# blink97/raytracing-gpu

Measured on AMD Instinct MI355X. Metric: Mrays/sec (primary+shadow) at 3840x2160, higher is better.
Workload: dtype f32; 1 GPU; C5 synthetic 10M-triangle sphere field (32x32 UV spheres of 53 stacks x 94 slices = 9776 tris + ground quad, seed 0x5EED, BASELINE.md), 3840x2160, device-built octree, exact camera rays (per-frame candidate lists); width=3840, height=2160, triangles=10010626, accel=octree_gpu

## Files before the change

### raytracing-gpu_amd/csrc/rt_ctx.h

```cpp
#pragma once
#include <hip/hip_runtime.h>
#include <rccl/rccl.h>

#include <algorithm>
#include <cerrno>
#include <chrono>
#include <cmath>
#include <cstdio>
#include <cstdlib>
#include <cstring>
#include <string>
#include <thread>
#include <vector>

#include "rt_build.h"
#include "rt_cand.h"
#include "rt_kernels.h"
#include "rt_forecast.h"
#include "rt_lightbuf.h"
#include "rt_mem.h"
#include "rt_relight.h"
#include "rt_shadow.h"
#include "rt_reflect.h"
#include "rt_tiles.h"

extern "C" {
#include "../host/rt_cull.h"
#include "../host/rt_internal.h"
}

#ifndef RT_EPS_ULPS_DEFAULT
#define RT_EPS_ULPS_DEFAULT 64
#endif
#ifndef RT_OOB_CAP
#define RT_OOB_CAP (1u << 20)
#endif
#ifndef RT_CAM_EPS_ULPS_DEFAULT
#define RT_CAM_EPS_ULPS_DEFAULT 64
#endif

#define HIP_TRY(expr)                                                                    \
  do {                                                                                   \
    hipError_t e_ = (expr);                                                              \
    if (e_ != hipSuccess)                                                                \
      return rt_set_error(RT_EHIP, "%s: %s (%s:%d)", #expr, hipGetErrorString(e_), __FILE__, \
                          __LINE__);                                                     \
  } while (0)

#define RT_TIMED_FRAMES 1024

static constexpr size_t kItemCounterBytes = 8 * 128;
static constexpr size_t kStatBytes = RT_STAT_SETS * RT_STAT_STRIDE * sizeof(unsigned long long);
static constexpr size_t kHitCounterBytes = 2 * RT_HIT_REGIONS * RT_HIT_STRIDE * sizeof(uint32_t);
static constexpr size_t kCostBytes = 64;
static constexpr size_t kFrameCounterBytes =
    kItemCounterBytes + kStatBytes + kHitCounterBytes + kCostBytes;

struct StreamOwner {
  hipStream_t s = nullptr;
  StreamOwner() = default;
  StreamOwner(const StreamOwner&) = delete;
  ~StreamOwner() { if (s) (void)hipStreamDestroy(s); }
  operator hipStream_t() const { return s; }
};

struct rt_hip_ctx {
  int device = 0;
  int accel = RT_ACCEL_FLAT;
  int count_work = 0;
  int grid = 0;
  StreamOwner stream;
  hipStream_t last_stream = nullptr;
  DevBuf<float4> d_tri;
  DevBuf<float> d_nrm;
  DevBuf<float> d_mat;
  DevBuf<float> d_light;
  DevBuf<float4> d_node;
  DevBuf<uint32_t> d_counter;
  unsigned long long* d_stats = nullptr;
  DevBuf<uint2> d_spill;
  uint32_t nrec = 0, nlight = 0;
  rt_accel_info info{};
  float scene_c[3]{}, scene_r = 0;
  float scene_lo[3]{}, scene_hi[3]{};
  float eps_ulps = RT_EPS_ULPS_DEFAULT;
  float cam_eps_ulps = RT_CAM_EPS_ULPS_DEFAULT;
  int policy = RT_POLICY_DEFAULT;
  DevBuf<unsigned long long> d_tile_cycles;
  DevBuf<float4> d_hit;
  DevBuf<uint32_t> d_hit_prev;
  DevBuf<float4> d_hit_term;
  uint32_t* d_hit_count = nullptr;
  size_t hit_cap() const {
    return std::min({d_hit.cap() / 2, d_hit_prev.cap(), d_hit_term.cap()}) / RT_HIT_REGIONS;
  }
  size_t hit_need = 0;
  DevBuf<uint32_t> d_last;
  int gbuffer = 0;
  DevBuf<uint4> d_capture;
  int gb_valid = 0;
  rt_frame gb_frame{};
  int keep_visibility = 0;
  DevBuf<uint32_t> d_hit_lit;
  RelightPlan relight;
  int rl_valid = 0;
  rt_frame rl_frame{};
  std::vector<float> mat_host;
#ifndef RT_ASYNC_LISTS_DEFAULT
#define RT_ASYNC_LISTS_DEFAULT 1
#endif
  int grid_of[2][RT_NPOLICIES][2] = {};
  int cus = 0;
  std::vector<uint32_t> light_type;
  std::vector<float> light_v;
  int light_buffers = 1;
  std::vector<LBDevice*> lb_dev;
  DevBuf<RtLightBuf> d_lbuf;
  std::vector<RtLightBuf> lb_host;
  std::vector<uint8_t> lb_failed;
  float lb_ulps = -1.0f;
  int lb_proven = -1;
  unsigned long long lb_entry_cap = 0;
  KParams last_p{};
  DevBuf<float2> d_prim_mu;
  DevBuf<float2> d_node_mu;
  DevBuf<uint4> d_oob;
  DevBuf<uint32_t> d_oob_count;
  DevBuf<unsigned long long> d_frame_check;
  DevBuf<uint32_t> d_sh_global;
  uint32_t n_sh_global = 0;
  int exact_refl = 0;
  DevBuf<float4> d_node_rf;
  unsigned long long rf_unbounded = 0;
  float sh_ulps = -1.0f;
  float sh_omax = 0.0f;
  float sh_mu_max = 1.0f;
  int exact_shadows = 1;
  size_t tile_cycles_n = 0;
  int exact_camera = 1;
#ifndef RT_CAND_REFINE_DEFAULT
#define RT_CAND_REFINE_DEFAULT 1
#endif
  int cand_refine = RT_CAND_REFINE_DEFAULT;
  const uint32_t* d_cand_valid = nullptr;
  double bound_scale = 1.0;
  float4* d_tri_prim = nullptr;
  DevBuf<float4> d_tri_prim_own;
  uint32_t nprim = 0;
  DevBuf<uint32_t> d_cand_list;
  DevBuf<void> d_cand_fp;
  DevBuf<uint4> d_cand_sfp;
  int cand_store_fp = 0;
  DevBuf<uint32_t> d_cand_visits;
  DevBuf<uint32_t> d_cand_off;
  DevBuf<uint32_t> d_cand_start;
  DevBuf<uint32_t> d_cand_keys;
  DevBuf<uint32_t> d_cand_keys2;
  DevBuf<uint32_t> d_cand_vals;
  DevBuf<uint32_t> d_cand_global;
  DevBuf<uint32_t> d_cand_big;
  DevBuf<uint32_t> d_cand_ctr;
  DevBuf<float> d_cand_skip;
  DevBuf<uint32_t> d_cand_big_lane;
  DevBuf<uint2> d_cand_items;
  DevBuf<uint32_t> d_cand_wave_items;
  DevBuf<uint32_t> d_cand_wave_base;
  DevBuf<uint32_t> d_scan_bsum;
  uint32_t cand_item_cap = 0xffffffffu;
  DevBuf<uint32_t> d_prim_leaf;
  DevBuf<uint32_t> d_cand;
  DevBuf<uint32_t> d_order;
  DevBuf<void> d_scan_tmp;
  PinnedBuf<uint32_t> h_cand;
  int async_lists = RT_ASYNC_LISTS_DEFAULT;
  ListForecast forecast;
  ListShape pknown;
  PinnedBuf<uint32_t> h_kept;
  hipEvent_t ev_kept = nullptr;
  ListShape cost_hist;
  uint32_t cost_waves = 0;
  DevBuf<uint32_t> d_item_cost;
  int last_async = 0;
  unsigned long long cand_prims = 0, cand_entries = 0, cand_global = 0;
  DevBuf<uint32_t> d_send;
  uint32_t send_n = 0;
  DevBuf<uint32_t> d_part;
  DevBuf<uint32_t> d_rstart;
  PinnedBuf<uint32_t> h_rstart;
  KParams ext{};
  int ext_ready = 0, ext_rank = -1, ext_nranks = 0;
  rt_frame ext_frame{};
  uint32_t ext_total = 0;
  int timing = 0;
  hipEvent_t ev[RT_TIMED_FRAMES][5] = {};
  unsigned long long frames = 0;

  ~rt_hip_ctx() {
    for (LBDevice* d : lb_dev) rt_lightbuf_free(d);
    if (ev_kept) (void)hipEventDestroy(ev_kept);
    for (auto& f : ev)
      for (hipEvent_t e : f)
        if (e) (void)hipEventDestroy(e);
  }
};

static inline void lists_changed(rt_hip_ctx* c) {
  c->forecast.reset();
  c->pknown.valid = 0;
}

static inline KParams scene_params(const rt_hip_ctx* c) {
  KParams p;
  std::memset(&p, 0, sizeof p);
  p.tri = c->d_tri;
  p.nrm = c->d_nrm;
  p.mat = c->d_mat;
  p.light = c->d_light;
  p.node = c->d_node;
  p.nrec = c->nrec;
  p.nlight = c->nlight;
  p.tri_prim = c->d_tri_prim;
  p.spill = c->d_spill;
  p.scene_c = rt::f3{c->scene_c[0], c->scene_c[1], c->scene_c[2]};
  p.scene_r = c->scene_r;
  p.scene_cmag = std::fmax(std::fabs(c->scene_c[0]), std::fmax(std::fabs(c->scene_c[1]),
                                                               std::fabs(c->scene_c[2])));
  p.eps_rel = c->eps_ulps * kSlackUnit;
  p.eps_rel_cam = c->cam_eps_ulps * kSlackUnit;
  return p;
}

static inline void scene_extent(const rt_flat_scene& fs, float c[3], float* r) {
  *r = 0;
  for (int a = 0; a < 3; a++) {
    float lo = fs.ntri ? fs.scene_lo[a] : 0.0f, hi = fs.ntri ? fs.scene_hi[a] : 0.0f;
    c[a] = 0.5f * (lo + hi);
    *r = std::fmax(*r, 0.5f * (hi - lo));
  }
}

int shadow_prepare(rt_hip_ctx* c, hipStream_t s);
int lbuf_prepare(rt_hip_ctx* c, hipStream_t s);
int reflect_prepare(rt_hip_ctx* c, hipStream_t s);
int choose_accel(const rt_scene* s);
int cand_prepare(rt_hip_ctx* c, const rt_frame* f, KParams* kp, hipStream_t s, int compat = 0);
unsigned long long* cost_sum_of(rt_hip_ctx* c);
```

### raytracing-gpu_amd/csrc/rt_hip.cpp

```cpp
#include "rt_ctx.h"

extern "C" int rt_hip_tiles_per_rank(int width, int height, int nranks) {
  if (width <= 0 || height <= 0 || nranks <= 0) return 0;
  const int tb = rt_block_side(nranks);
  return (int)(rt_max_rank_blocks((uint32_t)rt_blocks_x(tiles_x_of(width), tb),
                                  (uint32_t)rt_blocks_y(tiles_y_of(height), tb), (uint32_t)nranks) * tb * tb);
}

extern "C" size_t rt_hip_tile_buffer_floats(int width, int height, int nranks) {
  return (size_t)rt_hip_tiles_per_rank(width, height, nranks) * 64 * 3;
}

extern "C" int rt_hip_device_count(int* n) {
  if (!n) return rt_set_error(RT_EINVAL, "null argument");
  int c = 0;
  hipError_t e = hipGetDeviceCount(&c);
  if (e != hipSuccess || c <= 0) {
    *n = 0;
    return rt_set_error(RT_ENODEV, "no HIP device (%s)", hipGetErrorString(e));
  }
  *n = c;
  return RT_OK;
}

template <class T>
static int upload(DevBuf<T>& dst, const void* src, size_t bytes) {
  HIP_TRY(dst.alloc(bytes / sizeof(T)));
  if (src && bytes) HIP_TRY(hipMemcpy(dst, src, bytes, hipMemcpyHostToDevice));
  return RT_OK;
}

extern "C" void rt_hip_destroy(rt_hip_ctx* c) {
  if (!c) return;
  (void)hipSetDevice(c->device);
  delete c;
}

int shadow_prepare(rt_hip_ctx* c, hipStream_t s) {
  if (!c->exact_shadows || c->accel != RT_ACCEL_OCTREE || !c->d_node) return RT_OK;
  if (c->d_node_mu && c->sh_ulps == c->eps_ulps) return RT_OK;
  const size_t np = c->nprim, nn = c->info.nodes;
  if (!c->d_node_mu) {
    HIP_TRY(c->d_prim_mu.alloc(np + 1));
    HIP_TRY(c->d_sh_global.alloc(np + 1));
    HIP_TRY(c->d_node_mu.alloc(nn + 1));
  }
  DevBuf<uint32_t> d_n;
  HIP_TRY(d_n.alloc(1));
  ShadowParams sp;
  std::memset(&sp, 0, sizeof sp);
  sp.tri = c->d_tri_prim;
  sp.nprim = c->nprim;
  sp.light = c->d_light;
  sp.nlight = c->nlight;
  sp.node = c->d_node;
  sp.nnode = (uint32_t)nn;
  sp.rec = c->d_tri;
  for (int a = 0; a < 3; a++) sp.c[a] = c->scene_c[a];
  sp.R = c->scene_r;
  sp.eps_rel = (double)(c->eps_ulps * kSlackUnit);
  const double cmag = std::fmax(std::fabs(c->scene_c[0]), std::fmax(std::fabs(c->scene_c[1]),
                                                                  std::fabs(c->scene_c[2])));
  sp.plane_eps = (double)RT_CULL_PLANE * (cmag + c->scene_r) + 1e-6;
  sp.omax_assumed = 2.0 * c->scene_r + 1.0;
  sp.reach_cap = c->scene_r + 1.0;
  sp.prim_mu = c->d_prim_mu;
  sp.node_mu = c->d_node_mu;
  sp.global = c->d_sh_global;
  sp.nglobal = d_n;
  uint32_t n = 0;
  std::vector<float2> nm(1);
  HIP_TRY(hipMemsetAsync(d_n, 0, sizeof(uint32_t), s));
  HIP_TRY(rt_shadow_build(&sp, (int)c->info.max_depth + 2, s));
  HIP_TRY(hipMemcpyAsync(&n, d_n, sizeof n, hipMemcpyDeviceToHost, s));
  HIP_TRY(hipMemcpyAsync(nm.data(), c->d_node_mu, sizeof(float2), hipMemcpyDeviceToHost, s));
  HIP_TRY(hipStreamSynchronize(s));
  c->n_sh_global = n;
  c->sh_omax = (float)(sp.omax_assumed * (1.0 - 1e-6));
  c->sh_mu_max = nm[0].x;
  c->sh_ulps = c->eps_ulps;
  c->info.shadow_global = n;
  c->info.shadow_mu_max = nm[0].x;
  return RT_OK;
}

static void lbuf_release(rt_hip_ctx* c) {
  for (LBDevice*& d : c->lb_dev) {
    rt_lightbuf_free(d);
    d = nullptr;
  }
  c->d_lbuf.reset();
  c->lb_ulps = -1.0f;
}

static int lbuf_build_one(rt_hip_ctx* c, uint32_t li, hipStream_t s) {
  std::memset(&c->lb_host[li], 0, sizeof(RtLightBuf));
  c->lb_failed[li] = 0;
  const uint32_t t = c->light_type[li];
  if (t != 1 && t != 2) return RT_OK;
  char err[256] = {0};
  LBParams lp;
  lb_fill(lp, c->scene_c, c->scene_r, c->scene_lo, c->scene_hi, c->eps_ulps, t, &c->light_v[3 * li], c->nprim,
          c->exact_shadows);
  lp.tri = c->d_tri_prim;
  lp.max_entries = c->lb_entry_cap;
  if (const char* e = std::getenv("RT_LB_CELLS")) {
    const double k = std::atof(e);
    if (k > 0.0) lp.target_cells = (uint32_t)std::fmin((double)(1u << 26), std::fmax(4096.0, lp.target_cells * k));
  }
  const int br = rt_lightbuf_build(&lp, &c->lb_host[li], &c->lb_dev[li], s, err, sizeof err);
  if (br < 0) {
    (void)hipGetLastError();
    return rt_set_error(RT_EHIP, "light buffer of light %u: %s", li, err);
  }
  if (br > 0) {
    std::memset(&c->lb_host[li], 0, sizeof(RtLightBuf));
    c->lb_dev[li] = nullptr;
    (void)hipGetLastError();
    std::snprintf(c->info.lightbuf_fail_reason, sizeof c->info.lightbuf_fail_reason, "light %u: %s", li, err);
    c->lb_failed[li] = 1;
  }
  return RT_OK;
}

static int lbuf_publish(rt_hip_ctx* c) {
  uint32_t failed = 0;
  for (uint8_t f : c->lb_failed) failed += f;
  c->info.lightbuf_failed = failed;
  if (!failed) c->info.lightbuf_fail_reason[0] = 0;
  if (c->d_lbuf.cap() != c->lb_host.size() || !c->d_lbuf) HIP_TRY(c->d_lbuf.alloc(c->lb_host.size()));
  HIP_TRY(hipMemcpy(c->d_lbuf, c->lb_host.data(), c->lb_host.size() * sizeof(RtLightBuf), hipMemcpyHostToDevice));
  c->lb_ulps = c->eps_ulps;
  c->lb_proven = c->exact_shadows;
  unsigned long long e = 0, n = 0, g = 0, te = 0, tg = 0, nv = 0, bd = 0, tnv = 0, tbd = 0;
  for (LBDevice* d : c->lb_dev) {
    rt_lightbuf_sizes(d, &e, &n, &g);
    rt_lightbuf_proof_counts(d, &nv, &bd);
    te += e;
    tg += g;
    tnv += nv;
    tbd += bd;
  }
  c->info.lightbuf_entries = te;
  c->info.lightbuf_global = tg;
  c->info.lightbuf_never = tnv;
  c->info.lightbuf_band = tbd;
  return RT_OK;
}

int lbuf_prepare(rt_hip_ctx* c, hipStream_t s) {
  if (!c->light_buffers || c->accel != RT_ACCEL_OCTREE || !c->d_node || !c->nlight) return RT_OK;
  if (c->d_lbuf && c->lb_ulps == c->eps_ulps && c->lb_proven == c->exact_shadows) return RT_OK;
  lbuf_release(c);
  c->lb_dev.assign(c->nlight, nullptr);
  c->lb_host.assign(c->nlight, RtLightBuf{});
  c->lb_failed.assign(c->nlight, 0);
  c->info.lightbuf_fail_reason[0] = 0;
  for (uint32_t li = 0; li < c->nlight; li++) {
    const int rc = lbuf_build_one(c, li, s);
    if (rc) {
      for (LBDevice*& d : c->lb_dev) {
        rt_lightbuf_free(d);
        d = nullptr;
      }
      return rc;
    }
  }
  return lbuf_publish(c);
}

extern "C" int rt_hip_set_light_buffers(rt_hip_ctx* c, int enable) {
  if (!c) return rt_set_error(RT_EINVAL, "null context");
  c->light_buffers = enable ? 1 : 0;
  c->relight.invalidate();
  if (!c->light_buffers) lbuf_release(c);
  return RT_OK;
}

extern "C" int rt_hip_set_lightbuf_entry_cap(rt_hip_ctx* c, unsigned long long cap) {
  if (!c) return rt_set_error(RT_EINVAL, "null context");
  c->lb_entry_cap = cap;
  c->relight.invalidate();
  lbuf_release(c);
  HIP_TRY(hipSetDevice(c->device));
  return lbuf_prepare(c, c->stream);
}

extern "C" int rt_hip_create(int device, const rt_scene* scene, int accel, rt_hip_ctx** out) {
  if (!scene || !out) return rt_set_error(RT_EINVAL, "null argument");
  if (accel != RT_ACCEL_FLAT && accel != RT_ACCEL_OCTREE && accel != RT_ACCEL_OCTREE_GPU)
    return rt_set_error(RT_EINVAL, "unknown accel %d", accel);
  const bool dev_build = accel == RT_ACCEL_OCTREE_GPU;
  int ndev = 0;
  int rc = rt_hip_device_count(&ndev);
  if (rc) return rc;
  if (device < 0 || device >= ndev) return rt_set_error(RT_ENODEV, "device %d of %d", device, ndev);
  hipDeviceProp_t prop;
  HIP_TRY(hipGetDeviceProperties(&prop, device));
  if (std::strncmp(prop.gcnArchName, "gfx950", 6) != 0)
    return rt_set_error(RT_ENODEV, "device %d is %s, kernels are built for gfx950", device,
                        prop.gcnArchName);
  HIP_TRY(hipSetDevice(device));

  auto t0 = std::chrono::steady_clock::now();
  rt_flat_scene fs;
  rc = rt_flatten(scene, dev_build ? RT_ACCEL_FLAT : accel, &fs);
  if (rc) return rc;
  auto t1 = std::chrono::steady_clock::now();

  rt_hip_ctx* c = new rt_hip_ctx();
  if (const char* e = std::getenv("RT_CAND_REFINE")) c->cand_refine = std::atoi(e) != 0;
  if (const char* e = std::getenv("RT_ASYNC_LISTS")) c->async_lists = std::atoi(e) != 0;
  c->device = device;
  c->accel = dev_build ? (fs.ntri ? RT_ACCEL_OCTREE : RT_ACCEL_FLAT) : accel;
  c->nrec = (uint32_t)fs.nrec;
  c->nlight = (uint32_t)fs.nlight;
  size_t bytes_tri = fs.nrec * RT_TRI_FLOATS * sizeof(float);
  size_t bytes_nrm = fs.ntri * 9 * sizeof(float);
  size_t bytes_mat = fs.nobj * RT_MAT_FLOATS * sizeof(float);
  size_t bytes_light = fs.nlight * RT_LIGHT_FLOATS * sizeof(float);
  size_t bytes_node = fs.nnode * RT_NODE_FLOATS * sizeof(float);
  rc = upload(c->d_tri, fs.tri, bytes_tri);
  if (!rc) rc = upload(c->d_nrm, fs.nrm, bytes_nrm);
  if (!rc) rc = upload(c->d_mat, fs.mat, bytes_mat);
  if (!rc) rc = upload(c->d_light, fs.light, bytes_light);
  if (!rc && fs.nnode) rc = upload(c->d_node, fs.node, bytes_node);
  if (!rc) rc = upload(c->d_counter, nullptr, kFrameCounterBytes);
  if (!rc) {
    c->d_stats = (unsigned long long*)((char*)c->d_counter.get() + kItemCounterBytes);
    c->d_hit_count = (uint32_t*)((char*)c->d_counter.get() + kItemCounterBytes + kStatBytes);
  }
  if (!rc && hipStreamCreateWithFlags(&c->stream.s, hipStreamNonBlocking) != hipSuccess)
    rc = rt_set_error(RT_EHIP, "hipStreamCreate");
  rt_device_tree tree{};
  if (!rc && dev_build && fs.ntri) {
    rt_device_build_opts o{24, 7};
    if (const char* e = std::getenv("RT_DEV_LEAF")) o.leaf_cap = std::atoi(e);
    if (const char* e = std::getenv("RT_DEV_CLIP")) o.clip_level = std::atoi(e);
    hipError_t he = rt_device_build_octree(c->d_tri, (uint32_t)fs.ntri, fs.scene_lo, fs.scene_hi,
                                           &o, c->stream, &tree);
    if (he != hipSuccess) {
      rc = rt_set_error(RT_EHIP, "device octree build: %s", hipGetErrorString(he));
    } else {
      c->d_tri_prim_own = std::move(c->d_tri);
      c->d_tri_prim = c->d_tri_prim_own;
      c->d_tri.adopt(tree.tri, (size_t)tree.nref * RT_TRI_FLOATS / 4);
      c->d_node.adopt(tree.node, (size_t)tree.nnode * RT_NODE_FLOATS / 4);
      c->nrec = tree.nref;
      bytes_tri = (size_t)tree.nref * RT_TRI_FLOATS * sizeof(float);
      bytes_node = (size_t)tree.nnode * RT_NODE_FLOATS * sizeof(float);
      fs.nrec = tree.nref;
      fs.nnode = tree.nnode;
      fs.leaves = tree.leaves;
      fs.max_depth = tree.depth;
      fs.max_leaf = tree.max_leaf;
    }
  }
  auto t2 = std::chrono::steady_clock::now();
  c->nprim = (uint32_t)fs.ntri;
  if (!rc && !c->d_tri_prim) {
    if (c->accel == RT_ACCEL_FLAT) {
      c->d_tri_prim = c->d_tri;
    } else {
      rt_flat_scene fp;
      rc = rt_flatten(scene, RT_ACCEL_FLAT, &fp);
      if (!rc) {
        rc = upload(c->d_tri_prim_own, fp.tri, fp.nrec * RT_TRI_FLOATS * sizeof(float));
        c->d_tri_prim = c->d_tri_prim_own;
        rt_flat_free(&fp);
      }
    }
  }
  scene_extent(fs, c->scene_c, &c->scene_r);
  for (int a = 0; a < 3; a++) {
    c->scene_lo[a] = fs.ntri ? fs.scene_lo[a] : 0.0f;
    c->scene_hi[a] = fs.ntri ? fs.scene_hi[a] : 0.0f;
  }
  c->info.triangles = fs.ntri;
  c->info.tri_refs = fs.nrec;
  c->info.nodes = fs.nnode;
  c->info.leaves = fs.leaves;
  c->info.max_depth = fs.max_depth;
  c->info.max_leaf = fs.max_leaf;
  c->info.tri_record_bytes = RT_TRI_FLOATS * sizeof(float);
  c->info.node_record_bytes = RT_NODE_FLOATS * sizeof(float);
  c->info.device_bytes = bytes_tri + bytes_nrm + bytes_mat + bytes_light + bytes_node;
  c->info.build_seconds = std::chrono::duration<double>(dev_build ? t2 - t0 : t1 - t0).count();
  if (fs.mat) c->mat_host.assign(fs.mat, fs.mat + fs.nobj * RT_MAT_FLOATS);
  rt_flat_free(&fs);
  if (rc) {
    rt_hip_destroy(c);
    return rc;
  }
  c->grid = prop.multiProcessorCount * 16;
  c->cus = prop.multiProcessorCount;
  for (size_t li = 0; li < scene->light_count; li++) {
    c->light_type.push_back((uint32_t)scene->lights[li].type);
    c->light_v.push_back(scene->lights[li].v.x);
    c->light_v.push_back(scene->lights[li].v.y);
    c->light_v.push_back(scene->lights[li].v.z);
  }
  int gmax = c->grid;
  const int dacc = c->accel == RT_ACCEL_FLAT ? RT_ACCEL_FLAT_D : RT_ACCEL_OCTREE_D;
  for (int tr = 0; tr < 2; tr++)
    for (int pol = 0; pol < RT_NPOLICIES; pol++)
      for (int cw = 0; cw < 2; cw++) {
        int g = 0;
        hipError_t he = rt_render_grid(tr, dacc, cw, pol, prop.multiProcessorCount, &g);
        if (he != hipSuccess) {
          rt_hip_destroy(c);
          return rt_set_error(RT_EHIP, "occupancy query: %s", hipGetErrorString(he));
        }
        c->grid_of[tr][pol][cw] = g;
        gmax = g > gmax ? g : gmax;
      }
  c->info.trace_grid = c->grid_of[1][RT_POLICY_DEFAULT][0];
  c->info.shade_grid = c->grid_of[0][RT_POLICY_LBUF][0];
  for (int a = 0; a < 3; a++) c->info.scene_center[a] = c->scene_c[a];
  c->info.scene_radius = c->scene_r;
  if (c->accel == RT_ACCEL_OCTREE &&
      c->d_spill.alloc((size_t)gmax * 64 * RT_SPILL_STACK) != hipSuccess) {
    rt_hip_destroy(c);
    return rt_set_error(RT_EHIP, "hipMalloc traversal spill stack");
  }
  {
    const auto l0 = std::chrono::steady_clock::now();
    rc = lbuf_prepare(c, c->stream);
    c->info.lightbuf_seconds = std::chrono::duration<double>(std::chrono::steady_clock::now() - l0).count();
    if (rc) {
      rt_hip_destroy(c);
      return rc;
    }
  }
  *out = c;
  return RT_OK;
}

extern "C" int rt_hip_accel_info(const rt_hip_ctx* c, rt_accel_info* out) {
  if (!c || !out) return rt_set_error(RT_EINVAL, "null argument");
  *out = c->info;
  return RT_OK;
}

extern "C" int rt_hip_set_cull_slack(rt_hip_ctx* c, float ulps) {
  if (!c || !(ulps >= 0.0f)) return rt_set_error(RT_EINVAL, "bad slack");
  c->eps_ulps = ulps;
  c->cam_eps_ulps = ulps;
  c->relight.invalidate();
  lists_changed(c);
  return RT_OK;
}

extern "C" int rt_hip_set_camera_slack(rt_hip_ctx* c, float ulps) {
  if (!c || !(ulps >= 0.0f)) return rt_set_error(RT_EINVAL, "bad slack");
  c->cam_eps_ulps = ulps;
  lists_changed(c);
  return RT_OK;
}

extern "C" int rt_hip_set_exact_camera(rt_hip_ctx* c, int enable) {
  if (!c) return rt_set_error(RT_EINVAL, "null context");
  c->exact_camera = enable ? 1 : 0;
  return RT_OK;
}

extern "C" int rt_hip_set_exact_shadows(rt_hip_ctx* c, int enable) {
  if (!c) return rt_set_error(RT_EINVAL, "null context");
  c->exact_shadows = enable ? 1 : 0;
  c->relight.invalidate();
  HIP_TRY(hipSetDevice(c->device));
  int rc = lbuf_prepare(c, c->stream);
  if (rc) return rc;
  if (c->exact_shadows) return shadow_prepare(c, c->stream);
  return RT_OK;
}

static int reflect_build(rt_hip_ctx* c, hipStream_t s) {
  const size_t nn = c->info.nodes;
  DevBuf<float> phi;
  DevBuf<uint32_t> d_u;
  HIP_TRY(c->d_node_rf.alloc(3 * nn + 3));
  HIP_TRY(phi.alloc(nn + 1));
  HIP_TRY(d_u.alloc(1));
  ReflParams rp;
  std::memset(&rp, 0, sizeof rp);
  rp.node = c->d_node;
  rp.nnode = (uint32_t)nn;
  rp.rec = c->d_tri;
  rp.node_rf = c->d_node_rf;
  rp.node_phi = phi;
  rp.unbounded = d_u;
  uint32_t u = 0;
  HIP_TRY(hipMemsetAsync(c->d_node_rf, 0, (3 * nn + 3) * sizeof(float4), s));
  HIP_TRY(hipMemsetAsync(d_u, 0, sizeof(uint32_t), s));
  HIP_TRY(rt_reflect_build(&rp, (int)c->info.max_depth + 2, s));
  HIP_TRY(hipMemcpyAsync(&u, d_u, sizeof u, hipMemcpyDeviceToHost, s));
  HIP_TRY(hipStreamSynchronize(s));
  c->rf_unbounded = u;
  return RT_OK;
}

int reflect_prepare(rt_hip_ctx* c, hipStream_t s) {
  if (c->d_node_rf || c->accel != RT_ACCEL_OCTREE || !c->d_node) return RT_OK;
  const int rc = reflect_build(c, s);
  if (rc) c->d_node_rf.reset();
  return rc;
}

extern "C" int rt_hip_set_exact_reflections(rt_hip_ctx* c, int enable) {
  if (!c) return rt_set_error(RT_EINVAL, "null context");
  c->exact_refl = enable ? 1 : 0;
  if (!c->exact_refl) return RT_OK;
  HIP_TRY(hipSetDevice(c->device));
  return reflect_prepare(c, c->stream);
}

extern "C" int rt_hip_set_policy(rt_hip_ctx* c, int policy) {
  if (!c) return rt_set_error(RT_EINVAL, "null context");
  if (policy < RT_POLICY_DEFAULT || policy > RT_POLICY_DIR_STAGED)
    return rt_set_error(RT_EINVAL, "unknown traversal policy %d", policy);
  c->policy = policy;
  c->relight.invalidate();
  return RT_OK;
}

extern "C" int rt_hip_set_camera_refine(rt_hip_ctx* c, int enable) {
  if (!c) return rt_set_error(RT_EINVAL, "null context");
  c->cand_refine = enable ? 1 : 0;
  lists_changed(c);
  return RT_OK;
}

extern "C" int rt_hip_set_camera_bound_scale(rt_hip_ctx* c, double scale) {
  if (!c || !(scale > 0.0)) return rt_set_error(RT_EINVAL, "bad bound scale");
  c->bound_scale = scale;
  lists_changed(c);
  return RT_OK;
}

static int mask_buffer(rt_hip_ctx* c) {
  const size_t n = c->hit_cap() * RT_HIT_REGIONS;
  if (c->d_hit_lit.holds(n)) return RT_OK;
  c->relight.invalidate();
  HIP_TRY(c->d_hit_lit.alloc(n));
  return RT_OK;
}

static int hit_buffers(rt_hip_ctx* c, size_t ntiles) {
  const size_t items = 4 * ntiles;
  HIP_TRY(c->d_last.grow(items * 64, items * 64));
  if (c->gbuffer) HIP_TRY(c->d_capture.grow(items * 64, items * 64));
  size_t want =(2 * items * 64 + RT_HIT_REGIONS - 1) / RT_HIT_REGIONS + 1024;
  if (c->hit_need > want) want = c->hit_need;
  if (want > (1ull << 29) - 1) want = (1ull << 29) - 1;
  if (want <= c->hit_cap()) return c->keep_visibility ? mask_buffer(c) : RT_OK;
  c->d_hit.reset();
  c->d_hit_prev.reset();
  c->d_hit_term.reset();
  c->d_hit_lit.reset();
  c->relight.invalidate();
  const size_t n = want * RT_HIT_REGIONS;
  HIP_TRY(c->d_hit.alloc(2 * n));
  HIP_TRY(c->d_hit_prev.alloc(n));
  HIP_TRY(c->d_hit_term.alloc(n));
  return c->keep_visibility ? mask_buffer(c) : RT_OK;
}


static int render_refuse(const rt_hip_ctx* c, const rt_frame* f, int rank, int nranks, const float* d_tiles) {
  if (!c || !f || !d_tiles) return rt_set_error(RT_EINVAL, "null argument");
  if (nranks <= 0 || rank < 0 || rank >= nranks)
    return rt_set_error(RT_EINVAL, "rank %d of %d", rank, nranks);
  if (f->width <= 0 || f->height <= 0) return rt_set_error(RT_EINVAL, "empty frame");
  if ((f->width | f->height) & 1)
    return rt_set_error(RT_EINVAL, "frame %dx%d: cpu/rt renders even sizes only", f->width, f->height);
  if (c->gbuffer) {
    if (c->policy != RT_POLICY_DEFAULT)
      return rt_set_error(RT_EINVAL, "the G-buffer needs the default traversal policy (have %d)", c->policy);
    if (c->count_work) return rt_set_error(RT_EINVAL, "the G-buffer cannot be captured by the work-counting pass");
    if (c->exact_refl) return rt_set_error(RT_EINVAL, "the G-buffer cannot be captured with exact reflections on");
  }
  return RT_OK;
}

static void render_frame_params(KParams& p, const rt_hip_ctx* c, const rt_frame* f, int rank, int nranks,
                                float* d_tiles) {
  p.u = rt::f3{f->u.x, f->u.y, f->u.z};
  p.v = rt::f3{f->v.x, f->v.y, f->v.z};
  p.C = rt::f3{f->C.x, f->C.y, f->C.z};
  p.pos = rt::f3{f->position.x, f->position.y, f->position.z};
  p.W = f->width;
  p.H = f->height;
  p.tiles_x = tiles_x_of(f->width);
  p.ntiles_total = tiles_x_of(f->width) * tiles_y_of(f->height);
  p.rank = rank;
  p.nranks = nranks;
  p.ntiles_local = rank_tile_count(f->width, f->height, rank, nranks);
  p.out = d_tiles;
  p.tile_counter = c->d_counter;
  p.stats = c->d_stats;
}

static int render_done(rt_hip_ctx* c, const KParams& p, const rt_frame* f, hipStream_t s, int first_ev) {
  c->last_p = p;
  if (c->gbuffer) {
    c->gb_frame = *f;
    c->gb_valid = 1;
  }
  c->rl_frame = *f;
  c->rl_valid = 1;
  if (p.hit_lit)
    c->relight.masks_written();
  else
    c->relight.invalidate();
  if (c->timing) {
    hipEvent_t* ev = c->ev[c->frames % RT_TIMED_FRAMES];
    for (int k = first_ev; k < 5; k++) HIP_TRY(hipEventRecord(ev[k], s));
    c->frames++;
  }
  c->last_stream = s;
  return RT_OK;
}

static int render_nothing(rt_hip_ctx* c, const KParams& p, const rt_frame* f, hipStream_t s) {
  c->cand_prims = c->cand_entries = c->cand_global = 0;
  c->d_cand_valid = nullptr;
  c->last_async = 0;
  if (c->timing) HIP_TRY(hipEventRecord(c->ev[c->frames % RT_TIMED_FRAMES][0], s));
  HIP_TRY(hipMemsetAsync(c->d_counter, 0, kFrameCounterBytes, s));
  c->cost_hist.valid = 0;
  return render_done(c, p, f, s, 1);
}

static int render_buffers(rt_hip_ctx* c, KParams& p) {
  {
    int rc = hit_buffers(c, (size_t)p.ntiles_local);
    if (rc) return rc;
  }
  if (c->gbuffer) p.capture = c->d_capture;
  if (c->keep_visibility) p.hit_lit = c->d_hit_lit;
  p.hit = c->d_hit;
  p.hit_prev = c->d_hit_prev;
  p.hit_term = c->d_hit_term;
  p.hit_count = c->d_hit_count;
  p.shade_counter = c->d_hit_count + RT_HIT_REGIONS * RT_HIT_STRIDE;
  p.hit_cap = (uint32_t)c->hit_cap();
  p.last = c->d_last;
  if (c->count_work) {
    const size_t items = 4 * (size_t)p.ntiles_local;
    HIP_TRY(c->d_tile_cycles.grow(6 * items, 6 * items));
    c->tile_cycles_n = items;
    p.tile_cycles = c->d_tile_cycles;
  }
  return RT_OK;
}

static int render_shadows(rt_hip_ctx* c, KParams& p, hipStream_t s) {
  {
    int rc = lbuf_prepare(c, s);
    if (rc) return rc;
    if (c->policy == RT_POLICY_DEFAULT || c->policy == RT_POLICY_LANE) p.lbuf = c->d_lbuf;
  }
  const bool walks = !p.lbuf || c->info.lightbuf_failed;
  if (walks) {
    int rc = shadow_prepare(c, s);
    if (rc) return rc;
  }
  if (p.lbuf && c->exact_shadows && c->nlight <= 32) {
    if (!c->d_oob) {
      HIP_TRY(c->d_oob_count.alloc(1));
      HIP_TRY(c->d_oob.alloc(RT_OOB_CAP));
    }
    p.oob = c->d_oob;
    p.oob_count = c->d_oob_count;
    p.oob_cap = RT_OOB_CAP;
    HIP_TRY(hipMemsetAsync(c->d_oob_count, 0, sizeof(uint32_t), s));
  }
  if (c->exact_shadows && walks) {
    p.node_mu = c->d_node_mu;
    p.sh_global = c->d_sh_global;
    p.n_sh_global = c->n_sh_global;
    p.sh_omax = c->sh_omax;
  }
  return RT_OK;
}

static int render_lists(rt_hip_ctx* c, const rt_frame* f, KParams& p, bool use_ext, hipStream_t s) {
  c->cand_prims = c->cand_entries = c->cand_global = 0;
  c->d_cand_valid = nullptr;
  if (c->timing) HIP_TRY(hipEventRecord(c->ev[c->frames % RT_TIMED_FRAMES][0], s));
  if (c->accel == RT_ACCEL_OCTREE && c->d_node && c->exact_camera) {
    if (use_ext) {
      p.cand_start = c->ext.cand_start;
      p.cand = c->ext.cand;
      p.cand_global = c->ext.cand_global;
      p.n_cand_global = c->ext.n_cand_global;
      p.cand_skip = c->ext.cand_skip;
      p.tile_order = c->ext.tile_order;
      p.n_heavy = c->ext.n_heavy;
      p.tri_prim = c->ext.tri_prim;
      c->cand_entries = c->ext_total;
      c->d_cand_valid = nullptr;
      c->cand_global = c->ext.n_cand_global;
      c->cand_prims = 0;
    } else {
      int rc = cand_prepare(c, f, &p, s);
      if (rc) return rc;
    }
  }
  if (!(c->accel == RT_ACCEL_OCTREE && c->d_node && c->exact_camera && !use_ext)) c->last_async = 0;
  return RT_OK;
}

struct RenderKernels {
  int dacc, tpol, spol, gt, gs;
};

static int render_kernels(rt_hip_ctx* c, KParams& p, hipStream_t s, RenderKernels* out) {
  const bool empty = c->accel == RT_ACCEL_OCTREE && !c->d_node;
  const int dacc = (c->accel == RT_ACCEL_FLAT || empty) ? RT_ACCEL_FLAT_D : RT_ACCEL_OCTREE_D;
  const int pol = dacc == RT_ACCEL_FLAT_D ? 0 : c->policy, cw = c->count_work ? 1 : 0;
  int spol = pol;
  if (dacc == RT_ACCEL_OCTREE_D && p.lbuf && !p.node_mu && !p.n_sh_global &&
      (pol == RT_POLICY_DEFAULT || pol == RT_POLICY_LANE)) {
    bool all = true;
    for (uint32_t li = 0; li < c->nlight && all; li++)
      if (c->light_type[li] == 1 || c->light_type[li] == 2) all = c->lb_dev[li] != nullptr;
    if (all) spol = RT_POLICY_LBUF;
  }
  int tpol = pol;
  if (dacc == RT_ACCEL_OCTREE_D && c->exact_refl) {
    if (pol != RT_POLICY_DEFAULT)
      return rt_set_error(RT_EINVAL, "exact reflections need the default traversal policy (have %d)", pol);
    int rc = reflect_prepare(c, s);
    if (rc) return rc;
    p.node_rf = c->d_node_rf;
    tpol = RT_POLICY_EXACT_REFL;
  }
  if (c->gbuffer) tpol = RT_POLICY_GBUFFER;
  int gt = empty ? c->grid : c->grid_of[1][tpol][cw], gs = empty ? c->grid : c->grid_of[0][spol][cw];
  {
    const long long items = 4ll * p.ntiles_local;
    if (items < gt) gt = (int)items;
    if (items < gs) gs = (int)items;
  }
  *out = RenderKernels{dacc, tpol, spol, gt, gs};
  return RT_OK;
}

static int render_launch(rt_hip_ctx* c, const rt_frame* f, int rank, int nranks, KParams& p,
                         const RenderKernels& k, hipStream_t s) {
  hipEvent_t* ev = c->ev[c->frames % RT_TIMED_FRAMES];
  if (!p.tri_prim && (p.lbuf || p.n_sh_global || p.cand_start))
    return rt_set_error(RT_EHIP, "render: prim-order records missing");
  if (!p.hit || !p.last || !p.out || (p.nrec && (!p.tri || !p.nrm)))
    return rt_set_error(RT_EHIP, "render: device buffers missing");
  if (c->gbuffer && !p.capture) return rt_set_error(RT_EHIP, "render: G-buffer capture buffer missing");
  if (p.tile_order) {
    const size_t items = 4 * (size_t)p.ntiles_local;
    if (!c->d_item_cost.holds(items)) {
      c->cost_hist.valid = 0;
      HIP_TRY(c->d_item_cost.grow(items, items));
    }
    p.item_cost = c->d_item_cost;
    p.cost_sum = cost_sum_of(c);
  }
  if (!c->d_frame_check) {
    HIP_TRY(c->d_frame_check.alloc(4));
    HIP_TRY(hipMemsetAsync(c->d_frame_check, 0, 4 * sizeof(unsigned long long), s));
  }
  p.frame_check = c->d_frame_check;
  p.list_flag = c->last_async ? c->d_cand_ctr + RT_CAND_CTR_SNAPSHOT + RT_CC_OVERFLOW : nullptr;
  HIP_TRY(hipMemsetAsync(c->d_counter, 0, kFrameCounterBytes, s));
  if (c->timing) HIP_TRY(hipEventRecord(ev[1], s));
  HIP_TRY(rt_launch_trace(&p, k.dacc, c->count_work, k.tpol, k.gt, s));
  if (p.item_cost) {
    c->cost_hist.set(f, rank, nranks);
    c->cost_waves = (uint32_t)k.gt;
  } else {
    c->cost_hist.valid = 0;
  }
  if (c->timing) HIP_TRY(hipEventRecord(ev[2], s));
  HIP_TRY(rt_launch_shade(&p, k.dacc, c->count_work, k.spol, k.gs, s));
  HIP_TRY(rt_launch_shade_fixup(&p, c->nprim, s));
  if (c->timing) HIP_TRY(hipEventRecord(ev[3], s));
  HIP_TRY(rt_launch_fold(&p, s));
  return RT_OK;
}

extern "C" int rt_hip_render(rt_hip_ctx* c, const rt_frame* f, int rank, int nranks,
                             float* d_tiles, void* stream) {
  int rc = render_refuse(c, f, rank, nranks, d_tiles);
  if (rc) return rc;
  c->gb_valid = 0;
  c->rl_valid = 0;
  HIP_TRY(hipSetDevice(c->device));
  hipStream_t s = stream ? (hipStream_t)stream : c->stream;
  const bool use_ext = c->ext_ready && c->ext_rank == rank && c->ext_nranks == nranks &&
                       std::memcmp(&c->ext_frame, f, sizeof *f) == 0;
  c->ext_ready = 0;
  KParams p = scene_params(c);
  render_frame_params(p, c, f, rank, nranks, d_tiles);
  if (p.ntiles_local == 0) return render_nothing(c, p, f, s);
  RenderKernels k;
  if ((rc = render_buffers(c, p)) || (rc = render_shadows(c, p, s)) || (rc = render_lists(c, f, p, use_ext, s)) ||
      (rc = render_kernels(c, p, s, &k)) || (rc = render_launch(c, f, rank, nranks, p, k, s)))
    return rc;
  return render_done(c, p, f, s, 4);
}

extern "C" int rt_hip_stats(rt_hip_ctx* c, rt_stats* out) {
  if (!c || !out) return rt_set_error(RT_EINVAL, "null argument");
  HIP_TRY(hipSetDevice(c->device));
  unsigned long long hs[RT_STAT_SETS * RT_STAT_STRIDE], h[RT_NSTATS];
  uint32_t hc[RT_HIT_REGIONS * RT_HIT_STRIDE];
  hipStream_t s = c->last_stream ? c->last_stream : c->stream;
  HIP_TRY(hipMemcpyAsync(hs, c->d_stats, sizeof hs, hipMemcpyDeviceToHost, s));
  HIP_TRY(hipMemcpyAsync(hc, c->d_hit_count, sizeof hc, hipMemcpyDeviceToHost, s));
  uint32_t valid = 0, actr[RT_CC_BUILD_WORDS] = {};
  if (c->d_cand_valid) HIP_TRY(hipMemcpyAsync(&valid, c->d_cand_valid, sizeof valid, hipMemcpyDeviceToHost, s));
  const int was_async = c->last_async;
  if (was_async)
    HIP_TRY(hipMemcpyAsync(actr, c->d_cand_ctr + RT_CAND_CTR_SNAPSHOT, sizeof actr, hipMemcpyDeviceToHost, s));
  HIP_TRY(hipStreamSynchronize(s));
  if (c->d_cand_valid) {
    c->cand_entries = valid;
    c->d_cand_valid = nullptr;
  }
  if (was_async) {
    c->last_async = 0;
    c->cand_global = actr[RT_CC_GLOBAL];
    if (actr[RT_CC_OVERFLOW]) {
      lists_changed(c);
      return rt_set_error(RT_EHITBUF, "%u candidate-list entries, %u expected: render again", actr[RT_CC_TOTAL],
                          c->forecast.known.total);
    }
  }
  for (int k = 0; k < RT_NSTATS; k++) {
    h[k] = 0;
    for (int set = 0; set < RT_STAT_SETS; set++) h[k] += hs[set * RT_STAT_STRIDE + k];
  }
  size_t need = 0;
  unsigned long long records = 0;
  for (int x = 0; x < RT_HIT_REGIONS; x++) {
    need = hc[RT_HIT_STRIDE * x] > need ? hc[RT_HIT_STRIDE * x] : need;
    records += hc[RT_HIT_STRIDE * x];
  }
  std::memset(out, 0, sizeof *out);
  for (int k = 0; k < RT_NSTATS; k++) out->*rt_stat_member[k] = h[k];
  out->camera = 4 * h[RT_ST_PIXELS];
  out->hit_records = records;
  out->cand_prims = c->cand_prims;
  out->cand_entries = c->cand_entries;
  out->cand_global = c->cand_global;
  if (need > c->hit_cap()) {
    c->hit_need = need + need / 4 + 1024;
    return rt_set_error(RT_EHITBUF, "%llu hit records, %zu per region held (grown to %zu: render again)",
                        records, c->hit_cap(), c->hit_need);
  }
  if (out->depth_overflow)
    return rt_set_error(RT_EDEPTH, "%llu paths overflowed the bounce limit or a traversal stack",
                        out->depth_overflow);
  if (out->zero_normal)
    return rt_set_error(RT_EZERONORMAL,
                        "%llu closest hits had an exactly zero interpolated normal (cpu/hit.c:79 "
                        "would skip those objects)",
                        out->zero_normal);
  if (out->shadow_zero_risk)
    return rt_set_error(RT_EZERONORMAL,
                        "%llu shadow rays hit an object whose interpolated normal can vanish "
                        "(cpu/hit.c:99 may skip it; early any-hit exit not proven exact)",
                        out->shadow_zero_risk);
  if (c->last_p.oob) {
    uint32_t q = 0;
    HIP_TRY(hipMemcpy(&q, c->d_oob_count, sizeof q, hipMemcpyDeviceToHost));
    out->shadow_deferred = q;
    if (q > RT_OOB_CAP)
      return rt_set_error(RT_EINEXACT, "%u shadow queries from off the exact mode's proof box, %u decided",
                          q, RT_OOB_CAP);
  }
  if (out->closest_unproven)
    return rt_set_error(RT_EINEXACT,
                        "%llu reflection rays with |d| past the exact reflection walk's bound "
                        "(csrc/rt_reflect.h RT_RF_DLMAX)", out->closest_unproven);
  if (out->shadow_unproven)
    return rt_set_error(RT_EINEXACT,
                        "%llu shadow rays left from beyond the extent the exact shadow mode's "
                        "bound assumes (csrc/rt_shadow.hip, csrc/rt_lightbuf.hip)",
                        out->shadow_unproven);
  if (c->accel == RT_ACCEL_OCTREE && c->d_node &&
      (!c->exact_camera || c->bound_scale < 1.0 || c->eps_ulps < RT_EPS_ULPS_DEFAULT))
    return rt_set_error(RT_EINEXACT,
                        "rendered with exact_camera=%d, camera bound scale %g, culling slack %g ulps "
                        "(defaults 1, 1, %d): cpu/rt parity not guaranteed",
                        c->exact_camera, c->bound_scale, (double)c->eps_ulps, RT_EPS_ULPS_DEFAULT);
  return RT_OK;
}

extern "C" int rt_hip_assemble(rt_hip_ctx* c, const rt_frame* f, const float* d_gathered,
                               int nranks, float* d_rgb, void* stream) {
  if (!c || !f || !d_gathered || !d_rgb || nranks <= 0)
    return rt_set_error(RT_EINVAL, "bad argument");
  HIP_TRY(hipSetDevice(c->device));
  hipStream_t s = stream ? (hipStream_t)stream : c->stream;
  int tx = tiles_x_of(f->width);
  int nt = tx * tiles_y_of(f->height);
  HIP_TRY(rt_launch_assemble(d_gathered, d_rgb, f->width, f->height, tx, nt, nranks,
                             rt_hip_tiles_per_rank(f->width, f->height, nranks), s));
  return RT_OK;
}

extern "C" int rt_hip_render_image(rt_hip_ctx* c, const rt_frame* f, float* h_rgb, rt_stats* st) {
  if (!c || !f || !h_rgb) return rt_set_error(RT_EINVAL, "null argument");
  HIP_TRY(hipSetDevice(c->device));
  size_t nt = rt_hip_tile_buffer_floats(f->width, f->height, 1);
  size_t npx = (size_t)f->width * f->height;
  DevBuf<float> d_tiles, d_rgb;
  HIP_TRY(d_tiles.alloc(nt));
  if (d_rgb.alloc(npx * 3) != hipSuccess) return rt_set_error(RT_EHIP, "hipMalloc image");
  rt_stats tmp;
  int rc = RT_OK;
  for (int attempt = 0; attempt < 3; attempt++) {
    rc = rt_hip_render(c, f, 0, 1, d_tiles, nullptr);
    if (!rc) rc = rt_hip_assemble(c, f, d_tiles, 1, d_rgb, nullptr);
    if (!rc && hipMemcpyAsync(h_rgb, d_rgb, npx * 3 * sizeof(float), hipMemcpyDeviceToHost,
                              c->stream) != hipSuccess)
      rc = rt_set_error(RT_EHIP, "D2H image");
    if (!rc) rc = rt_hip_stats(c, st ? st : &tmp);
    if (rc != RT_EHITBUF) break;
  }
  return rc;
}


static std::vector<RelightLight> light_table(const rt_hip_ctx* c) {
  std::vector<RelightLight> t(c->nlight);
  for (uint32_t li = 0; li < c->nlight; li++) t[li] = RelightLight(c->light_type[li], &c->light_v[3 * li]);
  return t;
}

static int relight_quiesce(rt_hip_ctx* c) {
  if (c->last_stream && c->last_stream != c->stream.s) HIP_TRY(hipStreamSynchronize(c->last_stream));
  HIP_TRY(hipStreamSynchronize(c->stream));
  return RT_OK;
}

extern "C" int rt_hip_set_lights(rt_hip_ctx* c, const rt_light* lights, size_t n) {
  if (!c || (n && !lights)) return rt_set_error(RT_EINVAL, "null argument");
  if (n > 0x7fffffffu / RT_LIGHT_FLOATS) return rt_set_error(RT_EINVAL, "%zu lights", n);
  HIP_TRY(hipSetDevice(c->device));
  int rc = relight_quiesce(c);
  if (rc) return rc;
  std::vector<float> rows(n * RT_LIGHT_FLOATS, 0.0f), lv(3 * n);
  std::vector<uint32_t> type(n);
  for (size_t li = 0; li < n; li++) {
    const rt_light& l = lights[li];
    float* L = &rows[RT_LIGHT_FLOATS * li];
    type[li] = (uint32_t)l.type;
    std::memcpy(&L[0], &type[li], sizeof(float));
    L[1] = l.r, L[2] = l.g, L[3] = l.b;
    L[4] = lv[3 * li] = l.v.x, L[5] = lv[3 * li + 1] = l.v.y, L[6] = lv[3 * li + 2] = l.v.z;
  }
  const std::vector<RelightLight> was = light_table(c);
  const size_t old_n = c->nlight;
  rc = upload(c->d_light, rows.data(), rows.size() * sizeof(float));
  if (rc) return rc;
  c->nlight = (uint32_t)n;
  c->light_type = type;
  c->light_v = lv;
  const std::vector<RelightLight> now = light_table(c);
  std::vector<uint8_t> rebuild, release;
  c->relight.set_lights(was, now, rebuild, release);
  bool edited = was.size() != now.size();
  for (size_t li = 0; li < now.size() && !edited; li++) edited = !now[li].same(was[li]);
  if (edited) c->sh_ulps = -1.0f;
  c->last_p.light = c->d_light;
  c->last_p.nlight = c->nlight;
  if (!(c->light_buffers && c->accel == RT_ACCEL_OCTREE && c->d_node)) return RT_OK;
  const bool current = c->d_lbuf && c->lb_ulps == c->eps_ulps && c->lb_proven == c->exact_shadows &&
                       c->lb_dev.size() == old_n && c->lb_host.size() == old_n && c->lb_failed.size() == old_n;
  if (!current || n == 0) {
    lbuf_release(c);
    c->lb_dev.clear();
    c->lb_host.clear();
    c->lb_failed.clear();
    c->last_p.lbuf = nullptr;
    c->info.lightbuf_entries = c->info.lightbuf_global = c->info.lightbuf_never = c->info.lightbuf_band = 0;
    c->info.lightbuf_failed = 0;
    c->info.lightbuf_fail_reason[0] = 0;
    rc = lbuf_prepare(c, c->stream);
    if (c->last_p.hit) c->last_p.lbuf = c->d_lbuf;
    return rc;
  }
  for (size_t li = 0; li < old_n; li++)
    if (release[li]) {
      rt_lightbuf_free(c->lb_dev[li]);
      c->lb_dev[li] = nullptr;
    }
  c->lb_dev.resize(n, nullptr);
  c->lb_host.resize(n, RtLightBuf{});
  c->lb_failed.resize(n, 0);
  for (uint32_t li = 0; li < n; li++) {
    if (!now[li].casts()) {
      c->lb_host[li] = RtLightBuf{};
      c->lb_failed[li] = 0;
    }
    if (!rebuild[li]) continue;
    rc = lbuf_build_one(c, li, c->stream);
    if (rc) {
      lbuf_release(c);
      c->last_p.lbuf = nullptr;
      return rc;
    }
  }
  rc = lbuf_publish(c);
  c->last_p.lbuf = c->last_p.lbuf ? c->d_lbuf.get() : nullptr;
  return rc;
}

extern "C" int rt_hip_set_materials(rt_hip_ctx* c, const rt_object* objects, size_t n) {
  if (!c || (n && !objects)) return rt_set_error(RT_EINVAL, "null argument");
  if (n * RT_MAT_FLOATS != c->mat_host.size())
    return rt_set_error(RT_EINVAL, "%zu objects, the context has %zu", n, c->mat_host.size() / RT_MAT_FLOATS);
  std::vector<float> rows(c->mat_host.size(), 0.0f);
  for (size_t o = 0; o < n; o++) {
    const rt_object& ob = objects[o];
    float* m = &rows[RT_MAT_FLOATS * o];
    m[0] = ob.ka.x, m[1] = ob.ka.y, m[2] = ob.ka.z;
    m[3] = ob.kd.x, m[4] = ob.kd.y, m[5] = ob.kd.z;
    m[6] = ob.ks.x, m[7] = ob.ks.y, m[8] = ob.ks.z;
    m[9] = ob.ns;
    m[10] = ob.nr;
    if (std::memcmp(&m[10], &c->mat_host[RT_MAT_FLOATS * o + 10], 2 * sizeof(float)) != 0)
      return rt_set_error(RT_EINVAL, "object %zu: nr %g differs from the context's %g (reflectivity changes the paths: "
                          "create a new context)", o, (double)ob.nr, (double)c->mat_host[RT_MAT_FLOATS * o + 10]);
  }
  if (!n) return RT_OK;
  HIP_TRY(hipSetDevice(c->device));
  const int rc = relight_quiesce(c);
  if (rc) return rc;
  HIP_TRY(hipMemcpy(c->d_mat, rows.data(), rows.size() * sizeof(float), hipMemcpyHostToDevice));
  c->mat_host = rows;
  return RT_OK;
}

extern "C" int rt_hip_set_keep_visibility(rt_hip_ctx* c, int enable) {
  if (!c) return rt_set_error(RT_EINVAL, "null context");
  c->keep_visibility = enable ? 1 : 0;
  return RT_OK;
}

extern "C" int rt_hip_relight(rt_hip_ctx* c, const rt_frame* f, int rank, int nranks, float* d_tiles,
                              void* stream) {
  if (!c || !f || !d_tiles) return rt_set_error(RT_EINVAL, "null argument");
  if (!c->rl_valid)
    return rt_set_error(RT_EINVAL, "no kept hit records: rt_hip_render first (rt_hip_render_compat keeps none)");
  const KParams& lp = c->last_p;
  if (lp.rank != rank || lp.nranks != nranks || std::memcmp(&c->rl_frame, f, sizeof *f) != 0)
    return rt_set_error(RT_EINVAL, "the kept records are another frame's (last render: %dx%d, rank %d of %d)", lp.W,
                        lp.H, lp.rank, lp.nranks);
  hipStream_t s = stream ? (hipStream_t)stream : c->stream;
  if (s != c->last_stream) return rt_set_error(RT_EINVAL, "a relight runs on the stream of its render");
  if (c->policy != RT_POLICY_DEFAULT)
    return rt_set_error(RT_EINVAL, "a relight needs the default traversal policy (have %d)", c->policy);
  if (c->count_work) return rt_set_error(RT_EINVAL, "a relight cannot run as the work-counting pass");
  if (lp.ntiles_local == 0) return RT_OK;
  HIP_TRY(hipSetDevice(c->device));
  KParams p = lp;
  {
    const KParams sp = scene_params(c);
    p.light = sp.light;
    p.nlight = sp.nlight;
    p.mat = sp.mat;
    p.eps_rel = sp.eps_rel;
    p.eps_rel_cam = sp.eps_rel_cam;
  }
  p.out = d_tiles;
  p.lbuf = nullptr;
  p.node_mu = nullptr;
  p.sh_global = nullptr;
  p.n_sh_global = 0;
  p.sh_omax = 0.0f;
  p.oob = nullptr;
  p.oob_count = nullptr;
  p.oob_cap = 0;
  p.shade_stride = p.shade_first = 0;
  p.relight_dirty = 0;
  p.frame_check = nullptr;
  p.list_flag = nullptr;
  int rc = mask_buffer(c);
  if (rc) return rc;
  p.hit_lit = c->d_hit_lit;
  RenderKernels k;
  if ((rc = render_shadows(c, p, s)) || (rc = render_kernels(c, p, s, &k))) return rc;
  const RelightWork w = c->relight.work(light_table(c));
  if (w.path == RT_RELIGHT_RECOLOUR) p.oob = nullptr;
  if (!p.tri_prim && (p.lbuf || p.n_sh_global)) return rt_set_error(RT_EHIP, "relight: prim-order records missing");
  if (!p.hit || !p.hit_prev || !p.hit_term || !p.hit_lit || !p.hit_count || !p.shade_counter || !p.stats ||
      !p.last || !p.out || (p.nlight && !p.light) || (p.nrec && (!p.tri || !p.nrm)) || !p.mat ||
      p.hit_cap != c->hit_cap() || !c->d_hit_lit.holds((size_t)p.hit_cap * RT_HIT_REGIONS))
    return rt_set_error(RT_EHIP, "relight: device buffers missing");
  HIP_TRY(rt_launch_relight_zero(&p, s));
  if (w.path == RT_RELIGHT_RECOLOUR) {
    HIP_TRY(rt_launch_recolour(&p, c->cus, s));
  } else if (w.path == RT_RELIGHT_PARTIAL) {
    p.relight_dirty = w.dirty;
    HIP_TRY(rt_launch_reshade(&p, k.dacc, k.spol, k.gs, s));
  } else {
    HIP_TRY(rt_launch_shade(&p, k.dacc, 0, k.spol, k.gs, s));
  }
  HIP_TRY(rt_launch_shade_fixup(&p, c->nprim, s));
  HIP_TRY(rt_launch_fold(&p, s));
  c->relight.masks_written();
  c->last_p = p;
  return RT_OK;
}

extern "C" int rt_hip_relight_image(rt_hip_ctx* c, const rt_frame* f, float* h_rgb, rt_stats* st) {
  if (!c || !f || !h_rgb) return rt_set_error(RT_EINVAL, "null argument");
  if (f->width <= 0 || f->height <= 0) return rt_set_error(RT_EINVAL, "empty frame");
  HIP_TRY(hipSetDevice(c->device));
  const size_t nt = rt_hip_tile_buffer_floats(f->width, f->height, 1);
  const size_t npx = (size_t)f->width * f->height;
  DevBuf<float> d_tiles, d_rgb;
  HIP_TRY(d_tiles.alloc(nt));
  if (d_rgb.alloc(npx * 3) != hipSuccess) return rt_set_error(RT_EHIP, "hipMalloc image");
  rt_stats tmp;
  int rc = rt_hip_relight(c, f, 0, 1, d_tiles, nullptr);
  if (rc) return rc;
  rc = rt_hip_assemble(c, f, d_tiles, 1, d_rgb, nullptr);
  if (!rc && hipMemcpyAsync(h_rgb, d_rgb, npx * 3 * sizeof(float), hipMemcpyDeviceToHost, c->stream) != hipSuccess)
    rc = rt_set_error(RT_EHIP, "D2H image");
  const int src = rt_hip_stats(c, st ? st : &tmp);
  return rc ? rc : src;
}

static_assert(RT_GB_WORDS == RT_GB_WORDS_D && sizeof(rt_gsample) == 4 * RT_GB_WORDS,
              "rt_gsample is the record gbuffer_kernel writes");
extern "C" int rt_hip_set_gbuffer(rt_hip_ctx* c, int enable) {
  if (!c) return rt_set_error(RT_EINVAL, "null context");
  c->gbuffer = enable ? 1 : 0;
  if (!c->gbuffer) c->gb_valid = 0;
  return RT_OK;
}

extern "C" size_t rt_hip_gbuffer_tile_words(int width, int height, int nranks) {
  return (size_t)rt_hip_tiles_per_rank(width, height, nranks) * 64 * 4 * RT_GB_WORDS;
}

extern "C" int rt_hip_gbuffer(rt_hip_ctx* c, const rt_frame* f, int rank, int nranks, void* d_tiles,
                              void* stream) {
  if (!c || !f || !d_tiles) return rt_set_error(RT_EINVAL, "null argument");
  if ((uintptr_t)d_tiles & 7) return rt_set_error(RT_EINVAL, "G-buffer tiles must be 8-byte aligned");
  if (!c->gbuffer || !c->gb_valid)
    return rt_set_error(RT_EINVAL, "no G-buffer capture: rt_hip_set_gbuffer(1), then rt_hip_render");
  const KParams& lp = c->last_p;
  if (lp.rank != rank || lp.nranks != nranks || std::memcmp(&c->gb_frame, f, sizeof *f) != 0)
    return rt_set_error(RT_EINVAL, "the G-buffer holds another frame (last render: %dx%d, rank %d of %d)",
                        lp.W, lp.H, lp.rank, lp.nranks);
  hipStream_t s = stream ? (hipStream_t)stream : c->stream;
  if (s != c->last_stream)
    return rt_set_error(RT_EINVAL, "the G-buffer must be read on the stream of its render");
  if (lp.ntiles_local == 0) return RT_OK;
  HIP_TRY(hipSetDevice(c->device));
  if (!lp.capture || !lp.hit || (lp.nrec && !lp.tri_prim))
    return rt_set_error(RT_EHIP, "G-buffer: device buffers missing");
  HIP_TRY(rt_launch_gbuffer(&lp, (uint32_t*)d_tiles, s));
  return RT_OK;
}

extern "C" int rt_hip_assemble_gbuffer(rt_hip_ctx* c, const rt_frame* f, const void* d_gathered, int nranks,
                                       void* d_samples, void* stream) {
  if (!c || !f || !d_gathered || !d_samples || nranks <= 0) return rt_set_error(RT_EINVAL, "bad argument");
  if (f->width <= 0 || f->height <= 0) return rt_set_error(RT_EINVAL, "empty frame");
  HIP_TRY(hipSetDevice(c->device));
  hipStream_t s = stream ? (hipStream_t)stream : c->stream;
  HIP_TRY(rt_launch_assemble_words((const uint32_t*)d_gathered, (uint32_t*)d_samples, f->width, f->height,
                                   tiles_x_of(f->width), nranks,
                                   rt_hip_tiles_per_rank(f->width, f->height, nranks), 4 * RT_GB_WORDS, s));
  return RT_OK;
}

extern "C" int rt_hip_render_image_gbuffer(rt_hip_ctx* c, const rt_frame* f, float* h_rgb,
                                           rt_gsample* h_samples, rt_stats* st) {
  if (!c || !f || !h_rgb || !h_samples) return rt_set_error(RT_EINVAL, "null argument");
  if (f->width <= 0 || f->height <= 0) return rt_set_error(RT_EINVAL, "empty frame");
  HIP_TRY(hipSetDevice(c->device));
  const size_t nt = rt_hip_tile_buffer_floats(f->width, f->height, 1);
  const size_t ng = rt_hip_gbuffer_tile_words(f->width, f->height, 1);
  const size_t npx = (size_t)f->width * f->height;
  const size_t nsw = npx * 4 * RT_GB_WORDS;
  DevBuf<float> d_tiles, d_rgb;
  DevBuf<uint32_t> d_gt, d_gs;
  if (d_tiles.alloc(nt) != hipSuccess || d_rgb.alloc(npx * 3) != hipSuccess || d_gt.alloc(ng) != hipSuccess ||
      d_gs.alloc(nsw) != hipSuccess)
    return rt_set_error(RT_EHIP, "hipMalloc image and G-buffer");
  int rc = RT_OK;
  const int was = c->gbuffer;
  c->gbuffer = 1;
  rt_stats tmp;
  for (int attempt = 0; attempt < 3; attempt++) {
    rc = rt_hip_render(c, f, 0, 1, d_tiles, nullptr);
    if (!rc) rc = rt_hip_assemble(c, f, d_tiles, 1, d_rgb, nullptr);
    if (!rc) rc = rt_hip_gbuffer(c, f, 0, 1, d_gt, nullptr);
    if (!rc) rc = rt_hip_assemble_gbuffer(c, f, d_gt, 1, d_gs, nullptr);
    if (!rc && (hipMemcpyAsync(h_rgb, d_rgb, npx * 3 * sizeof(float), hipMemcpyDeviceToHost, c->stream) !=
                    hipSuccess ||
                hipMemcpyAsync(h_samples, d_gs, nsw * sizeof(uint32_t), hipMemcpyDeviceToHost, c->stream) !=
                    hipSuccess))
      rc = rt_set_error(RT_EHIP, "D2H image and G-buffer");
    if (!rc) rc = rt_hip_stats(c, st ? st : &tmp);
    if (rc != RT_EHITBUF) break;
  }
  c->gbuffer = was;
  if (!was) c->gb_valid = 0;
  return rc;
}

int choose_accel(const rt_scene* s);

extern "C" int rt_hip_render_compat(rt_hip_ctx* c, const rt_camera* cam, unsigned char* h_rgba,
                                    rt_stats* st) {
  if (!c || !cam || !h_rgba) return rt_set_error(RT_EINVAL, "null argument");
  if (cam->width <= 0 || cam->height <= 0) return rt_set_error(RT_EINVAL, "empty frame");
  if ((long long)cam->width * cam->height > (1ll << 28) / 9)
    return rt_set_error(RT_EINVAL, "frame too large for the 3x render");
  HIP_TRY(hipSetDevice(c->device));
  rt_camera big = *cam;
  big.width = 3 * cam->width;
  big.height = 3 * cam->height;
  rt_frame f;
  int rc = rt_frame_from_camera_any(&big, &f);
  if (rc) return rc;
  const size_t nhi = (size_t)big.width * big.height, nlo = (size_t)cam->width * cam->height;
  DevBuf<uint32_t> d_hi, d_lo;
  HIP_TRY(d_hi.alloc(nhi));
  if (d_lo.alloc(nlo) != hipSuccess) return rt_set_error(RT_EHIP, "hipMalloc image");
  hipStream_t s = c->stream;
  KParams p = scene_params(c);
  p.u = rt::f3{f.u.x, f.u.y, f.u.z};
  p.v = rt::f3{f.v.x, f.v.y, f.v.z};
  p.C = rt::f3{f.C.x, f.C.y, f.C.z};
  p.pos = rt::f3{f.position.x, f.position.y, f.position.z};
  p.W = big.width;
  p.H = big.height;
  p.tiles_x = tiles_x_of(big.width);
  p.ntiles_total = tiles_x_of(big.width) * tiles_y_of(big.height);
  p.nranks = 1;
  p.ntiles_local = p.ntiles_total;
  p.out = (float*)d_hi.get();
  p.tile_counter = c->d_counter;
  p.stats = c->d_stats;
  const int accel = (c->accel == RT_ACCEL_FLAT || !c->d_node) ? RT_ACCEL_FLAT_D : RT_ACCEL_OCTREE_D;
  rc = shadow_prepare(c, s);
  if (rc) return rc;
  if (c->exact_shadows) {
    p.node_mu = c->d_node_mu;
    p.sh_global = c->d_sh_global;
    p.n_sh_global = c->n_sh_global;
    p.sh_omax = c->sh_omax;
  }
  c->cand_prims = c->cand_entries = c->cand_global = 0;
  c->d_cand_valid = nullptr;
  if (c->accel == RT_ACCEL_OCTREE && c->d_node && c->exact_camera) {
    rc = cand_prepare(c, &f, &p, s, 1);
    if (rc) return rc;
  }
  c->cost_hist.valid = 0;
  c->rl_valid = 0;
  c->relight.invalidate();
  if (hipMemsetAsync(c->d_counter, 0, kFrameCounterBytes, s) != hipSuccess ||
      rt_launch_compat(&p, accel, c->grid, s) != hipSuccess ||
      rt_launch_downscale(d_hi, d_lo, cam->width, cam->height, s) != hipSuccess ||
      hipMemcpyAsync(h_rgba, d_lo, nlo * sizeof(uint32_t), hipMemcpyDeviceToHost, s) != hipSuccess)
    rc = rt_set_error(RT_EHIP, "compat render: %s", hipGetErrorString(hipGetLastError()));
  c->last_stream = s;
  rt_stats tmp;
  if (!rc) rc = rt_hip_stats(c, st ? st : &tmp);
  if (st) st->camera = st->pixels;
  return rc;
}

extern "C" int rt_raytrace_gpu(const char* input, const char* output, int accel) {
  rt_scene* scene = nullptr;
  int rc = rt_scene_load_svati(input, &scene);
  if (rc) return rc;
  if (accel < 0) accel = choose_accel(scene);
  rt_hip_ctx* ctx = nullptr;
  std::vector<unsigned char> img((size_t)4 * (scene->camera.width > 0 ? scene->camera.width : 0) *
                                 (scene->camera.height > 0 ? scene->camera.height : 0) + 4);
  rc = rt_hip_create(0, scene, accel, &ctx);
  if (!rc) rc = rt_hip_render_compat(ctx, &scene->camera, img.data(), nullptr);
  if (!rc) rc = rt_png_write_rgba(output, scene->camera.width, scene->camera.height, img.data());
  if (ctx) rt_hip_destroy(ctx);
  rt_scene_free(scene);
  return rc;
}

extern "C" int rt_hip_malloc(int device, size_t bytes, void** d_ptr) {
  if (!d_ptr) return rt_set_error(RT_EINVAL, "null argument");
  HIP_TRY(hipSetDevice(device));
  HIP_TRY(hipMalloc(d_ptr, bytes ? bytes : 16));
  return RT_OK;
}
extern "C" int rt_hip_free(void* d_ptr) {
  HIP_TRY(hipFree(d_ptr));
  return RT_OK;
}
extern "C" int rt_hip_memcpy_d2h(void* dst, const void* src, size_t bytes) {
  HIP_TRY(hipMemcpy(dst, src, bytes, hipMemcpyDeviceToHost));
  return RT_OK;
}
extern "C" int rt_hip_memcpy_h2d(void* dst, const void* src, size_t bytes) {
  HIP_TRY(hipMemcpy(dst, src, bytes, hipMemcpyHostToDevice));
  return RT_OK;
}

extern "C" int rt_hip_memcpy_d2d(void* dst, const void* src, size_t bytes, void* stream) {
  if (!bytes) return RT_OK;
  HIP_TRY(hipMemcpyAsync(dst, src, bytes, hipMemcpyDeviceToDevice, (hipStream_t)stream));
  return RT_OK;
}


int choose_accel(const rt_scene* s) {
  size_t n = rt_scene_triangle_count(s);
  return n <= 64 ? RT_ACCEL_FLAT : (n < 100000 ? RT_ACCEL_OCTREE : RT_ACCEL_OCTREE_GPU);
}

extern "C" int rt_raytrace(const char* input, const char* output) {
  return rt_raytrace_multi(input, output, 1, -1, nullptr, nullptr);
}
```

### raytracing-gpu_amd/csrc/rt_isect.h

```cpp
#pragma once

#include <hip/hip_runtime.h>
#include <stdint.h>

#include "rt_cull.h"
#include "rt_device.h"
#include "rt_kernels.h"

namespace rt {

static constexpr float kEps = 0.0000001f;

__device__ __forceinline__ void wave_sync() { __asm__ volatile("" ::: "memory"); }
__device__ __forceinline__ uint64_t wave_ballot(bool p) { return __builtin_amdgcn_ballot_w64(p); }

__device__ __forceinline__ f3 ld3(const float* p) { return f3{p[0], p[1], p[2]}; }

__device__ __forceinline__ bool mt_test(f3 o, f3 d, f3 v0, f3 e1, f3 e2, float& t, float& u,
                                        float& v) {
  f3 h = cross(d, e2);
  float a = dot(e1, h);
  if (a > -kEps && a < kEps) return false;
  float f = 1.0f / a;
  f3 s = sub(o, v0);
  u = f * dot(s, h);
  if (u < 0.0f || u > 1.0f) return false;
  f3 q = cross(s, e1);
  v = f * dot(d, q);
  if (v < 0.0f || u + v > 1.0f) return false;
  t = f * dot(e2, q);
  return t > kEps;
}

struct Ray {
  f3 o, d;
  float dlen;
  float eps;
  f3 oh, ol;
};

__device__ __forceinline__ Ray make_ray(const KParams& p, f3 o, f3 d, float eps_rel) {
  Ray r;
  r.o = o;
  r.d = d;
  r.dlen = length(d);
  r.eps = rt_cull_eps(eps_rel, o.x - p.scene_c.x, o.y - p.scene_c.y, o.z - p.scene_c.z,
                      p.scene_cmag, p.scene_r);
  r.oh = f3{o.x + r.eps, o.y + r.eps, o.z + r.eps};
  r.ol = f3{o.x - r.eps, o.y - r.eps, o.z - r.eps};
  return r;
}

__device__ __forceinline__ f3 hit_point(const Ray& r, float t) {
  f3 nd{r.d.x / r.dlen, r.d.y / r.dlen, r.d.z / r.dlen};
  return add(r.o, scale(nd, t * r.dlen));
}

__device__ __forceinline__ float hit_dist(const Ray& r, float t) {
  return length(sub(hit_point(r, t), r.o));
}

__device__ __forceinline__ bool mt_candidate(f3 o, f3 d, f3 v0, f3 e1, f3 e2, float t_cut) {
  const float m = 1e-5f;
  f3 h = cross(d, e2);
  float a = dot(e1, h);
  if (a > -kEps && a < kEps) return false;
  float r = __builtin_amdgcn_rcpf(a);
  f3 s = sub(o, v0);
  float u = dot(s, h) * r;
  if (u < -1e-30f || u > 1.0f + m) return false;
  f3 q = cross(s, e1);
  float v = dot(d, q) * r;
  if (v < -1e-30f || u + v > 1.0f + m) return false;
  float t = dot(e2, q) * r;
  return !(t < kEps * (1.0f - m) || t > t_cut);
}

__device__ __forceinline__ void mt_candidate2(f3 o, f3 d, const float4* qa, const float4* qb,
                                              float t_cut, bool& ca, bool& cb) {
  const float m = 1e-5f;
  const f3 v0a{qa[0].x, qa[0].y, qa[0].z}, e1a{qa[0].w, qa[1].x, qa[1].y}, e2a{qa[1].z, qa[1].w, qa[2].x};
  const f3 v0b{qb[0].x, qb[0].y, qb[0].z}, e1b{qb[0].w, qb[1].x, qb[1].y}, e2b{qb[1].z, qb[1].w, qb[2].x};
  const f3 ha = cross(d, e2a), hb = cross(d, e2b);
  const float aa = dot(e1a, ha), ab = dot(e1b, hb);
  const float ra = __builtin_amdgcn_rcpf(aa), rb = __builtin_amdgcn_rcpf(ab);
  const f3 sa = sub(o, v0a), sb = sub(o, v0b);
  const float ua = dot(sa, ha) * ra, ub = dot(sb, hb) * rb;
  ca = !(aa > -kEps && aa < kEps) && !(ua < -1e-30f || ua > 1.0f + m);
  cb = !(ab > -kEps && ab < kEps) && !(ub < -1e-30f || ub > 1.0f + m);
  if (__ballot(ca || cb) == 0) return;
  const f3 qva = cross(sa, e1a), qvb = cross(sb, e1b);
  const float va = dot(d, qva) * ra, vb = dot(d, qvb) * rb;
  ca = ca && !(va < -1e-30f || ua + va > 1.0f + m);
  cb = cb && !(vb < -1e-30f || ub + vb > 1.0f + m);
  if (__ballot(ca || cb) == 0) return;
  const float ta = dot(e2a, qva) * ra, tb = dot(e2b, qvb) * rb;
  ca = ca && !(ta < kEps * (1.0f - m) || ta > t_cut);
  cb = cb && !(tb < kEps * (1.0f - m) || tb > t_cut);
}

struct Best {
  float dist;
  float t_cut;
  uint32_t prim, obj;
  float u, v;
  float t;
};

__device__ __forceinline__ void consider_exact(const Ray& r, const float4& q0, const float4& q1,
                                               const float4& q2, Best& b);

__device__ __forceinline__ void consider(const Ray& r, const float4& q0, const float4& q1,
                                         const float4& q2, Best& b) {
  f3 v0{q0.x, q0.y, q0.z}, e1{q0.w, q1.x, q1.y}, e2{q1.z, q1.w, q2.x};
  if (!mt_candidate(r.o, r.d, v0, e1, e2, b.t_cut)) return;
  consider_exact(r, q0, q1, q2, b);
}

__device__ __forceinline__ void consider_exact(const Ray& r, const float4& q0, const float4& q1,
                                               const float4& q2, Best& b) {
  f3 v0{q0.x, q0.y, q0.z}, e1{q0.w, q1.x, q1.y}, e2{q1.z, q1.w, q2.x};
  float t, u, v;
  if (!mt_test(r.o, r.d, v0, e1, e2, t, u, v)) return;
  float nd = hit_dist(r, t);
  if (!((double)nd > 0.01)) return;
  uint32_t prim = __float_as_uint(q2.y);
  if (nd < b.dist || (nd == b.dist && prim < b.prim)) {
    b.dist = nd;
    float ao = fmaxf(fabsf(r.o.x), fmaxf(fabsf(r.o.y), fabsf(r.o.z)));
    b.t_cut = (nd * (1.0f + 1e-5f) + (ao + nd) * 2e-6f) / r.dlen;
    b.prim = prim;
    b.obj = __float_as_uint(q2.z);
    b.u = u;
    b.v = v;
    b.t = t;
  }
}

__device__ __forceinline__ void consider_w(const Ray& r, bool act, uint64_t am, const float4& q0,
                                           const float4& q1, const float4& q2, Best& b) {
  const float m = 1e-5f;
  const f3 v0{q0.x, q0.y, q0.z}, e1{q0.w, q1.x, q1.y}, e2{q1.z, q1.w, q2.x};
  const f3 h = cross(r.d, e2);
  const float a = dot(e1, h);
  const float rc = __builtin_amdgcn_rcpf(a);
  const f3 s = sub(r.o, v0);
  const float u = dot(s, h) * rc;
  const bool ca = !(a > -kEps && a < kEps), cu0 = !(u < -1e-30f), cu1 = !(u > 1.0f + m);
  bool c = act && ca && cu0 && cu1;
  if ((am & wave_ballot(ca) & wave_ballot(cu0) & wave_ballot(cu1)) == 0) return;
  const f3 q = cross(s, e1);
  const float v = dot(r.d, q) * rc;
  const float t = dot(e2, q) * rc;
  c = c && !(v < -1e-30f || u + v > 1.0f + m) && !(t < kEps * (1.0f - m) || t > b.t_cut);
  if (c) consider_exact(r, q0, q1, q2, b);
}

__device__ __forceinline__ void stage_test(const Ray& r, bool act, uint64_t am, uint32_t n, Best& b,
                                           const float4* stage) {
  uint32_t k3 = 0;
  __asm__ volatile("" : "+v"(k3));
  for (uint32_t k = 0; k < n; k++, k3 += 3) consider_w(r, act, am, stage[k3], stage[k3 + 1], stage[k3 + 2], b);
}

__device__ __forceinline__ bool any_hit_exact(const Ray& r, const float4& q0, const float4& q1,
                                              const float4& q2, uint32_t& risk);

__device__ __forceinline__ bool any_hit_rec(const Ray& r, const float4& q0, const float4& q1,
                                            const float4& q2, uint32_t& risk) {
  f3 v0{q0.x, q0.y, q0.z}, e1{q0.w, q1.x, q1.y}, e2{q1.z, q1.w, q2.x};
  if (!mt_candidate(r.o, r.d, v0, e1, e2, __builtin_inff())) return false;
  return any_hit_exact(r, q0, q1, q2, risk);
}

__device__ __forceinline__ bool any_hit_exact(const Ray& r, const float4& q0, const float4& q1,
                                              const float4& q2, uint32_t& risk) {
  f3 v0{q0.x, q0.y, q0.z}, e1{q0.w, q1.x, q1.y}, e2{q1.z, q1.w, q2.x};
  float t, u, v;
  if (!mt_test(r.o, r.d, v0, e1, e2, t, u, v)) return false;
  if (!((double)hit_dist(r, t) > 0.01)) return false;
  risk |= __float_as_uint(q2.w) & RT_REC_ZERO_RISK;
  return true;
}

}
```

### raytracing-gpu_amd/csrc/rt_kernels.h

```cpp
#pragma once

#include <hip/hip_runtime.h>
#include <stdint.h>

#include "rt_counters.h"
#include "rt_device.h"
#include "rt_lightbuf.h"

#define RT_ACCEL_FLAT_D 0
#define RT_ACCEL_OCTREE_D 1
#define RT_MAT_FLOATS_D 12
#define RT_LIGHT_FLOATS_D 8
#define RT_MAX_BOUNCES 16384
#define RT_SPILL_STACK 112
#define RT_HIT_REGIONS 8
#define RT_HIT_STRIDE 32
#define RT_NO_REC 0xffffffffu
#ifndef RT_MIN_WAVES
#define RT_MIN_WAVES 3
#endif
#ifndef RT_TRACE_MIN_WAVES
#define RT_TRACE_MIN_WAVES 5
#endif
#ifndef RT_SHADE_MIN_WAVES
#define RT_SHADE_MIN_WAVES 7
#endif
#ifndef RT_STAGED_SHADE_MIN_WAVES
#define RT_STAGED_SHADE_MIN_WAVES 4
#endif
#ifndef RT_FLAT_SHADE_MIN_WAVES
#define RT_FLAT_SHADE_MIN_WAVES 5
#endif
#define RT_REC_ZERO_RISK 1u
#define RT_POLICY_DEFAULT 0
#define RT_POLICY_LANE 1
#define RT_POLICY_STAGED 2
#define RT_POLICY_DIR_STAGED 3
#define RT_POLICY_LBUF 4
#define RT_POLICY_EXACT_REFL 5
#define RT_POLICY_GBUFFER 6
#define RT_NPOLICIES 7
#define RT_GB_WORDS_D 10

struct WorkCount {
  uint32_t closest, shadow, pixels, nodes, tris, overflow, zero_normal, hits;
  uint32_t cl_nodes, cl_tris, sh_nodes, sh_tris;
  uint32_t cy_cam, cy_cand, cy_sec, cy_shadow;
  uint32_t cy_shadow_dir;
  uint32_t stack_spills;
  uint32_t zero_risk;
  uint32_t sh_unproven;
  uint32_t cl_unproven;
  uint32_t sec_lane_nodes, sec_lane_tris;
};

struct KParams {
  const float4* tri;
  const float* nrm;
  const float* mat;
  const float* light;
  const float4* node;
  uint32_t nrec, nlight;
  rt::f3 u, v, C, pos;
  int W, H;
  int tiles_x, ntiles_total, rank, nranks, ntiles_local;
  float* out;
  float4* hit;
  uint32_t* hit_prev;
  float4* hit_term;
  uint32_t* hit_count;
  uint32_t hit_cap;
  uint32_t* last;
  uint32_t* shade_counter;
  uint32_t* hit_lit;
  uint32_t shade_stride;
  uint32_t shade_first;
  const RtLightBuf* lbuf;
  const float2* node_mu;
  const float4* node_rf;
  const uint32_t* sh_global;
  uint32_t n_sh_global;
  float sh_omax;
  uint4* oob;
  uint32_t* oob_count;
  uint32_t oob_cap;
  uint32_t* tile_counter;
  unsigned long long* stats;
  uint2* spill;
  rt::f3 scene_c;
  float scene_cmag;
  float scene_r;
  float eps_rel;
  float eps_rel_cam;
  unsigned long long* tile_cycles;
  const uint32_t* cand_start;
  const uint32_t* cand;
  const uint32_t* cand_global;
  uint32_t n_cand_global;
  const uint32_t* n_cand_global_dev;
  const float4* tri_prim;
  const float* cand_skip;
  const uint32_t* tile_order;
  uint32_t* item_cost;
  unsigned long long* cost_sum;
  const uint32_t* n_heavy;
  unsigned long long* frame_check;
  const uint32_t* list_flag;
  uint4* capture;
  uint32_t relight_dirty;
};

extern "C" hipError_t rt_launch_trace(const KParams* p, int accel, int count_work, int policy,
                                      int grid, hipStream_t stream);
extern "C" hipError_t rt_launch_shade(const KParams* p, int accel, int count_work, int policy,
                                      int grid, hipStream_t stream);
extern "C" hipError_t rt_launch_shade_fixup(const KParams* p, uint32_t nprim, hipStream_t stream);
extern "C" hipError_t rt_launch_fold(const KParams* p, hipStream_t stream);
extern "C" hipError_t rt_launch_relight_zero(const KParams* p, hipStream_t stream);
extern "C" hipError_t rt_launch_recolour(const KParams* p, int cus, hipStream_t stream);
extern "C" hipError_t rt_launch_reshade(const KParams* p, int accel, int policy, int grid, hipStream_t stream);
extern "C" hipError_t rt_launch_probe_shadow(const KParams* p, const float* org, uint32_t n, uint32_t li,
                                             uint32_t nprim, int brute, uint32_t* out, hipStream_t stream);
extern "C" hipError_t rt_launch_probe_closest(const KParams* p, const float* org, const float* dir, uint32_t n,
                                              uint32_t nprim, int brute, uint32_t* out, int grid, hipStream_t stream);
extern "C" hipError_t rt_render_grid(int trace, int accel, int count_work, int policy, int cus,
                                     int* grid);
extern "C" hipError_t rt_launch_compat(const KParams* p, int accel, int grid, hipStream_t stream);
extern "C" hipError_t rt_launch_downscale(const uint32_t* hi, uint32_t* lo, int W, int H,
                                          hipStream_t stream);
extern "C" hipError_t rt_launch_assemble(const float* tiles, float* rgb, int W, int H, int tiles_x,
                                         int ntiles, int nranks, int tiles_per_rank,
                                         hipStream_t stream);
extern "C" hipError_t rt_launch_gbuffer(const KParams* p, uint32_t* out, hipStream_t stream);
extern "C" hipError_t rt_launch_assemble_words(const uint32_t* tiles, uint32_t* out, int W, int H, int tiles_x,
                                               int nranks, int tiles_per_rank, int words,
                                               hipStream_t stream);
```

### raytracing-gpu_amd/csrc/rt_query.h

```cpp
#pragma once

#include "rt_lightbuf_cell.h"
#include "rt_walk_lane.h"
#include "rt_walk_wave.h"

namespace rt {

static constexpr int kPacketMin = 8;
#ifndef RT_PACKET_MAX_DEPTH
#define RT_PACKET_MAX_DEPTH 0
#endif
static constexpr int kPacketMaxDepth = RT_PACKET_MAX_DEPTH;

static constexpr int kTpMaxLanes = 48;
__device__ __forceinline__ bool use_tp(const KParams& p, bool act) {
  return p.nrec >= 256u && __popcll(__ballot(act)) <= kTpMaxLanes;
}

template <int ACCEL, bool COUNT, int POL>
__device__ __forceinline__ void closest_q(const KParams& p, const Ray& r, bool act, int depth, Best& b,
                                          Stack& s, WaveCtx& w, WorkCount& wc) {
  if (ACCEL == RT_ACCEL_FLAT_D) {
    if (use_tp(p, act))
      flat_closest_tp<COUNT>(p, r, act, b, wc);
    else
      flat_closest_w<COUNT>(p, r, act, b, w, wc);
    return;
  }
  if (POL == RT_POLICY_EXACT_REFL && depth > 0) {
    LaneCount lc = {0, 0, 0, 0, 0, 0, 0, 0};
    if (act) oct_closest_rf<COUNT>(p, r, b, s, lc);
    absorb<COUNT>(wc, lc, false);
    return;
  }
  bool staged = POL == RT_POLICY_STAGED ||
                (POL != RT_POLICY_LANE && __popcll(__ballot(act)) >= kPacketMin &&
                 depth <= kPacketMaxDepth);
  if (staged) {
    staged_closest<COUNT>(p, r, act, b, w, wc);
  } else {
    LaneCount lc = {0, 0, 0, 0, 0, 0, 0, 0};
    if (act) oct_closest<COUNT>(p, r, b, s, lc);
    absorb<COUNT>(wc, lc, false);
    if (COUNT && depth > 0) {
      uint32_t mn = lc.lnodes, mt = lc.ltris;
#pragma unroll
      for (int off = 32; off > 0; off >>= 1) {
        mn = max(mn, (uint32_t)__shfl_xor((int)mn, off));
        mt = max(mt, (uint32_t)__shfl_xor((int)mt, off));
      }
      wc.sec_lane_nodes = max(wc.sec_lane_nodes, uni(mn));
      wc.sec_lane_tris = max(wc.sec_lane_tris, uni(mt));
    }
  }
}

struct LbRange {
  uint32_t rs[2], re[2];
  float lim;
};

__device__ __forceinline__ LbRange lbuf_range(const RtLightBuf& L, const Ray& r) {
  uint32_t cell[2] = {0xffffffffu, 0xffffffffu};
  float lim = __builtin_inff();
  lbuf_cells(L, r.o, r.d, cell, lim);
  LbRange g;
  g.lim = lim;
  for (int h = 0; h < 2; h++) {
    g.rs[h] = 0u;
    g.re[h] = 0u;
    if (cell[h] != 0xffffffffu) {
      g.rs[h] = L.start[cell[h]];
      g.re[h] = L.start[cell[h] + 1];
    }
  }
  return g;
}

template <bool COUNT>
__device__ bool lbuf_scan(const KParams& p, const RtLightBuf& L, const Ray& r, const LbRange& g, LaneCount& lc) {
  for (int h = 0; h < 2; h++) {
    const float q = h == 0 ? g.lim : __builtin_inff();
    uint32_t k = g.rs[h];
    const uint32_t e = g.re[h];
    float4 n0, n1, n2;
    if (k < e) {
      const float4* t = L.rec + 3 * (size_t)k;
      n0 = t[0];
      n1 = t[1];
      n2 = t[2];
    }
    for (; k < e; k++) {
      const float4 a0 = n0, a1 = n1, a2 = n2;
      if (k + 1 < e) {
        const float4* t = L.rec + 3 * (size_t)(k + 1);
        n0 = t[0];
        n1 = t[1];
        n2 = t[2];
      }
      if (a2.y > q) break;
      if (COUNT) {
        lc.tris += lanes_distinct(k);
        lc.ltris++;
      }
      if (any_hit_rec(r, a0, a1, a2, lc.risk)) return true;
    }
  }
  for (uint32_t k = 0; k < L.nglobal; k++) {
    const float4* t = p.tri_prim + 3 * (size_t)L.global[k];
    if (COUNT) {
      lc.tris += lanes_distinct(L.global[k]);
      lc.ltris++;
    }
    if (any_hit_rec(r, t[0], t[1], t[2], lc.risk)) return true;
  }
  return false;
}

template <bool COUNT>
__device__ bool lbuf_any(const KParams& p, const RtLightBuf& L, const Ray& r, LaneCount& lc) {
  return lbuf_scan<COUNT>(p, L, r, lbuf_range(L, r), lc);
}

template <int ACCEL, bool COUNT, int POL>
__device__ __forceinline__ bool shadow_q(const KParams& p, f3 o, f3 d, uint32_t type, uint32_t li,
                                         bool act, Stack& s, WaveCtx& w, WorkCount& wc, bool* defer = nullptr,
                                         const LbRange* pre = nullptr, bool can_defer = true) {
  uint64_t am = __ballot(act);
  wc.shadow += (uint32_t)__popcll(am);
  Ray r = make_ray(p, o, d, p.eps_rel);
  if (ACCEL == RT_ACCEL_FLAT_D)
    return use_tp(p, act) ? flat_any_tp<COUNT>(p, r, act, wc) : flat_any_w<COUNT>(p, r, act, w, wc);
  if (POL == RT_POLICY_LBUF) {
    const RtLightBuf& L = p.lbuf[li];
    LaneCount lc = {0, 0, 0, 0, 0, 0, 0, 0};
    bool hit = act && (pre ? lbuf_scan<COUNT>(p, L, r, *pre, lc) : lbuf_any<COUNT>(p, L, r, lc));
    absorb<COUNT>(wc, lc, true);
    if (L.proven) {
      const bool out = act && !(o.x >= L.olo[0] && o.x <= L.ohi[0] && o.y >= L.olo[1] && o.y <= L.ohi[1] &&
                                o.z >= L.olo[2] && o.z <= L.ohi[2]);
      if (defer && can_defer && p.oob) {
        *defer = out;
        if (out) hit = false;
      } else {
        wc.sh_unproven += (uint32_t)__popcll(__ballot(out));
      }
    }
    return hit;
  }
  bool staged = POL == RT_POLICY_STAGED ||
                (POL == RT_POLICY_DIR_STAGED && type == 1 && __popcll(am) >= kPacketMin);
  bool hit, walked = true;
  if (staged) {
    hit = staged_any<COUNT>(p, r, act, w, wc);
  } else if (p.lbuf && p.lbuf[li].kind != RT_LB_NONE) {
    walked = false;
    const RtLightBuf& L = p.lbuf[li];
    LaneCount lc = {0, 0, 0, 0, 0, 0, 0, 0};
    hit = act && (pre ? lbuf_scan<COUNT>(p, L, r, *pre, lc) : lbuf_any<COUNT>(p, L, r, lc));
    absorb<COUNT>(wc, lc, true);
    if (L.proven) {
      const bool out = act && !(o.x >= L.olo[0] && o.x <= L.ohi[0] && o.y >= L.olo[1] && o.y <= L.ohi[1] &&
                                o.z >= L.olo[2] && o.z <= L.ohi[2]);
      if (defer && can_defer && p.oob) {
        *defer = out;
        if (out) hit = false;
      } else {
        wc.sh_unproven += (uint32_t)__popcll(__ballot(out));
      }
    }
  } else {
    LaneCount lc = {0, 0, 0, 0, 0, 0, 0, 0};
    hit = act && oct_any<COUNT>(p, r, s, lc);
    absorb<COUNT>(wc, lc, true);
  }
  if (walked && p.n_sh_global && __ballot(act && !hit)) {
    uint32_t risk = 0;
    for (uint32_t k = 0; k < p.n_sh_global; k++) {
      const float4* q = p.tri_prim + 3 * (size_t)uni(p.sh_global[k]);
      const float4 q0 = ldu(q, 0), q1 = ldu(q, 1), q2 = ldu(q, 2);
      if (act && !hit) hit = any_hit_rec(r, q0, q1, q2, risk);
      if (__ballot(act && !hit) == 0) break;
    }
    wc.zero_risk += (uint32_t)__popcll(__ballot(risk != 0));
  }
  if (walked && type == 2 && p.node_mu) {
    const float m = fmaxf(fabsf(o.x - p.scene_c.x), fmaxf(fabsf(o.y - p.scene_c.y), fabsf(o.z - p.scene_c.z)));
    wc.sh_unproven += (uint32_t)__popcll(__ballot(act && !(m <= p.sh_omax)));
  }
  return hit;
}

template <bool COUNT>
__device__ __forceinline__ uint32_t cand_range(const KParams& p, const Ray& r, bool act, uint32_t s, uint32_t e,
                                               float bmax, Best& b, WaveCtx& w) {
  const int lane = w.lane;
  const uint64_t am = wave_ballot(act);
  uint32_t tested = 0;
  for (uint32_t base = s; base < e; base += kOctRecs) {
    uint32_t prim = 0;
    bool keep = false;
    if (lane < kOctRecs && base + lane < e) {
      prim = p.cand[base + lane];
      keep = !(p.cand_skip[base + lane] > bmax);
    }
    const uint64_t m = wave_ballot(keep);
    if (m == 0) continue;
    const uint32_t n = (uint32_t)__popcll(m);
    const uint32_t slot = (uint32_t)__popcll(m & ((1ull << lane) - 1ull));
    float4 g0, g1, g2;
    if (keep) {
      const float4* q = p.tri_prim + 3 * (size_t)prim;
      g0 = q[0];
      g1 = q[1];
      g2 = q[2];
    }
    wave_sync();
    if (keep) {
      w.stage[3 * slot] = g0;
      w.stage[3 * slot + 1] = g1;
      w.stage[3 * slot + 2] = g2;
    }
    wave_sync();
    stage_test(r, act, am, n, b, w.stage);
    tested += n;
  }
  return tested;
}

template <bool COUNT>
__device__ __forceinline__ void cand_closest(const KParams& p, const Ray& r, bool act, uint32_t tile,
                                             Best& b, WaveCtx& w, WorkCount& wc) {
  if (!p.cand_start || __ballot(act) == 0) return;
    float bl = -__builtin_inff();
    if (act)
      bl = b.dist == __builtin_inff() ? __builtin_inff()
                                      : (b.dist - length(sub(p.pos, r.o))) + (2e-3f + 4e-7f * b.dist);
#pragma unroll
    for (int off = 32; off > 0; off >>= 1) bl = fmaxf(bl, __shfl_xor(bl, off));
    const float bmax = __uint_as_float(uni(__float_as_uint(bl)));
  const uint32_t tested =
      cand_range<COUNT>(p, r, act, uni(p.cand_start[tile]), uni(p.cand_start[tile + 1]), bmax, b, w);
  const uint32_t n_glob = p.n_cand_global_dev ? uni(*p.n_cand_global_dev) : p.n_cand_global;
  for (uint32_t k = 0; k < n_glob; k++) {
    const float4* q = p.tri_prim + 3 * (size_t)uni(p.cand_global[k]);
    float4 q0 = ldu(q, 0), q1 = ldu(q, 1), q2 = ldu(q, 2);
    if (act) consider(r, q0, q1, q2, b);
  }
  if (COUNT) {
    wc.tris += tested + n_glob;
    wc.cl_tris += (tested + n_glob) * (uint32_t)__popcll(__ballot(act));
  }
}

}
```

### raytracing-gpu_amd/csrc/rt_recolour.h

```cpp
#pragma once

#include "rt_shading.h"

namespace rt {

constexpr bool shade_stat_slot(uint32_t k) {
  return k == RT_ST_SHADOW || k == RT_ST_SHADOW_NODE_LANES || k == RT_ST_SHADOW_TRI_LANES ||
         k == RT_ST_CYCLES_SHADOW || k == RT_ST_CYCLES_SHADOW_DIRECTIONAL ||
         (k >= RT_ST_SHADOW_ZERO_RISK && k <= RT_ST_SHADOW_UNPROVEN);
}
constexpr bool shade_stat_slots_agree(uint32_t k = 0) {
  return k == RT_STAT_STRIDE || (shade_stat_slot(k) == rt_stat_shade_side(k) && shade_stat_slots_agree(k + 1));
}
static_assert(shade_stat_slots_agree(), "shade_stat_slot differs from the SHADE rows of RT_STAT_LIST");

template <int K = 0>
__global__ __launch_bounds__(256) void relight_zero_kernel(KParams p) {
  static_assert(RT_HIT_REGIONS * RT_HIT_STRIDE <= 256 && RT_STAT_SETS * RT_STAT_STRIDE <= 256,
                "one workgroup covers both");
  const uint32_t t = threadIdx.x;
  if (t < RT_HIT_REGIONS * RT_HIT_STRIDE) p.shade_counter[t] = 0u;
  if (t < RT_STAT_SETS * RT_STAT_STRIDE && shade_stat_slot(t % RT_STAT_STRIDE)) p.stats[t] = 0ull;
}

static constexpr uint32_t kRecolourLights = 64;

__device__ __forceinline__ col recolour_sum(const float* light, uint32_t nlight, uint32_t mask, const float* m,
                                            f3 P, f3 N) {
  col acc = init_color(0.0f, 0.0f, 0.0f);
  for (uint32_t l0 = 0; l0 < nlight; l0 += 32) {
    const uint32_t l1 = nlight - l0 < 32u ? nlight : l0 + 32u;
    acc = lights_sum(light, acc, l0, l1, l0 == 0 ? mask : 0u, m, P, N);
  }
  return acc;
}

template <int K = 0>
__global__ __launch_bounds__(256) void recolour_kernel(KParams p) {
  __shared__ float s_light[kRecolourLights * RT_LIGHT_FLOATS_D];
  const bool staged = p.nlight <= kRecolourLights;
  if (staged)
    for (uint32_t i = threadIdx.x; i < p.nlight * RT_LIGHT_FLOATS_D; i += blockDim.x) s_light[i] = p.light[i];
  __syncthreads();
  uint32_t end[RT_HIT_REGIONS];
  uint32_t total = 0;
#pragma unroll
  for (int x = 0; x < RT_HIT_REGIONS; x++) {
    const uint32_t hc = p.hit_count[RT_HIT_STRIDE * x];
    total += hc < p.hit_cap ? hc : p.hit_cap;
    end[x] = total;
  }
  const uint32_t nth = gridDim.x * blockDim.x;
  for (uint64_t g64 = blockIdx.x * blockDim.x + threadIdx.x; g64 < total; g64 += nth) {
    const uint32_t g = (uint32_t)g64;
    uint32_t x = 0, first = 0;
#pragma unroll
    for (int k = 0; k < RT_HIT_REGIONS - 1; k++)
      if (g >= end[k]) {
        x = k + 1;
        first = end[k];
      }
    const size_t a = (size_t)x * p.hit_cap + (g - first);
    const float4 r0 = p.hit[2 * a], r1 = p.hit[2 * a + 1];
    const uint32_t mask = p.hit_lit[a];
    const f3 P{r0.x, r0.y, r0.z}, N{r0.w, r1.x, r1.y};
    const float* m = p.mat + RT_MAT_FLOATS_D * (size_t)__float_as_uint(r1.w);
    const col local = staged ? recolour_sum(s_light, p.nlight, mask, m, P, N)
                             : recolour_sum(p.light, p.nlight, mask, m, P, N);
    const col tm = color_mul(local, r1.z);
    p.hit_term[a] = make_float4(tm.r, tm.g, tm.b, 0.0f);
  }
}

}
```

### raytracing-gpu_amd/csrc/rt_render.hip

```cpp
#include <hip/hip_runtime.h>
#include <stdint.h>

#include "rt_cull.h"
#include "rt_device.h"
#include "rt_kernels.h"
#include "rt_reflect.h"
#include "rt_tiles.h"

#include "rt_isect.h"
#include "rt_walk_lane.h"
#include "rt_walk_wave.h"
#include "rt_query.h"
#include "rt_shading.h"

namespace rt {

__device__ __forceinline__ void tile_pixel(const KParams& p, uint32_t t, int row, int col, int& pr,
                                           int& pc) {
  int tx, ty;
  const int tb = rt_block_side(p.nranks);
  rt_tile_xy(t, (uint32_t)p.rank, (uint32_t)p.nranks, (uint32_t)rt_blocks_x(p.tiles_x, tb), (uint32_t)tb,
             &tx, &ty);
  pr = ty * 8 + row;
  pc = tx * 8 + col;
}

__device__ __forceinline__ void flush_counts(const KParams& p, const WorkCount& wc, int lane,
                                             bool shade = false) {
  uint32_t v[RT_NSTATS];
  v[RT_ST_CLOSEST] = wc.closest, v[RT_ST_SHADOW] = wc.shadow, v[RT_ST_PIXELS] = wc.pixels;
  v[RT_ST_NODE_VISITS] = shade ? 0u : wc.nodes, v[RT_ST_TRI_TESTS] = shade ? 0u : wc.tris;
  v[RT_ST_DEPTH_OVERFLOW] = wc.overflow, v[RT_ST_ZERO_NORMAL] = wc.zero_normal, v[RT_ST_HITS] = wc.hits;
  v[RT_ST_CLOSEST_NODE_LANES] = wc.cl_nodes, v[RT_ST_CLOSEST_TRI_LANES] = wc.cl_tris;
  v[RT_ST_SHADOW_NODE_LANES] = wc.sh_nodes, v[RT_ST_SHADOW_TRI_LANES] = wc.sh_tris;
  v[RT_ST_CYCLES_CAMERA] = wc.cy_cam, v[RT_ST_CYCLES_CAND] = wc.cy_cand, v[RT_ST_CYCLES_SECONDARY] = wc.cy_sec;
  v[RT_ST_CYCLES_SHADOW] = wc.cy_shadow, v[RT_ST_CYCLES_SHADOW_DIRECTIONAL] = wc.cy_shadow_dir;
  v[RT_ST_STACK_SPILLS] = wc.stack_spills, v[RT_ST_SHADOW_ZERO_RISK] = wc.zero_risk;
  v[RT_ST_SHADOW_NODE_VISITS] = shade ? wc.nodes : 0u, v[RT_ST_SHADOW_TRI_TESTS] = shade ? wc.tris : 0u;
  v[RT_ST_SHADOW_UNPROVEN] = wc.sh_unproven, v[RT_ST_CLOSEST_UNPROVEN] = wc.cl_unproven;
#pragma unroll
  for (int k = 0; k < RT_NSTATS; k++)
    if (lane == 0 && v[k])
      atomicAdd(p.stats + (size_t)(blockIdx.x % RT_STAT_SETS) * RT_STAT_STRIDE + k, (unsigned long long)v[k]);
}


__device__ __forceinline__ size_t rec_addr(const KParams& p, uint32_t idx) {
  return (size_t)(idx & 7u) * p.hit_cap + (idx >> 3);
}

__device__ __forceinline__ bool camera_sample(const KParams& p, uint32_t t, uint32_t q, int lane, int& smp,
                                              f3& point, f3& dir) {
  int row, col, pr, pc;
  asm volatile("" : "+v"(lane));
  rt_item_pixel(q, (uint32_t)lane, &row, &col, &smp);
  tile_pixel(p, t, row, col, pr, pc);
  const int ii = p.W - pc, jj = p.H - pr;
  const bool valid = pr < p.H && pc < p.W && ii >= 1 && ii <= 2 * (p.W / 2) && jj >= 1 && jj <= 2 * (p.H / 2);
  const int i = ii - p.W / 2, j = jj - p.H / 2;
  const float k = (float)i + 0.5f * (float)(smp >> 1);
  const float l = (float)j + 0.5f * (float)(smp & 1);
  point = add(add(p.C, scale(p.u, k)), scale(p.v, l));
  dir = normalize(sub(p.pos, point));
  return valid;
}

struct Capture {
  uint32_t prim = 0xffffffffu;
  uint32_t dist = 0x7f800000u;
  uint32_t first = RT_NO_REC;
  uint32_t queries = 0;
};

template <int ACCEL, bool COUNT, int POL>
__device__ __forceinline__ uint32_t trace_path(const KParams& p, bool valid, f3 o, f3 d,
                                               uint32_t x, Stack& s, WaveCtx& w, WorkCount& wc,
                                               uint32_t tile, Capture& cap, int depth = 0, float coef = 1.0f,
                                               uint32_t prev = RT_NO_REC) {
  constexpr bool kCapture = POL == RT_POLICY_GBUFFER;
  bool alive = valid;
  for (;;) {
    alive = alive && !((double)coef < 0.01);
    uint64_t am = __ballot(alive);
    if (am == 0) break;
    wc.closest += (uint32_t)__popcll(am);
    if (kCapture && alive) cap.queries++;
    Ray r = make_ray(p, o, d, depth == 0 ? p.eps_rel_cam : p.eps_rel);
    Best b;
    b.dist = __builtin_inff();
    b.t_cut = __builtin_inff();
    b.prim = 0xffffffffu;
    b.obj = 0;
    b.u = b.v = 0.0f;
    b.t = 0.0f;
    uint64_t c0 = COUNT ? __builtin_readcyclecounter() : 0ull;
    closest_q<ACCEL, COUNT, POL>(p, r, alive, depth, b, s, w, wc);
    if (COUNT) {
      const uint64_t c1 = __builtin_readcyclecounter();
      (depth == 0 ? wc.cy_cam : wc.cy_sec) += (uint32_t)(c1 - c0);
      c0 = c1;
    }
    if (ACCEL != RT_ACCEL_FLAT_D && depth == 0) cand_closest<COUNT>(p, r, alive, tile, b, w, wc);
    if (COUNT) wc.cy_cand += (uint32_t)(__builtin_readcyclecounter() - c0);
    bool hit = alive && b.dist != __builtin_inff();
    if (kCapture && depth == 0 && hit) {
      cap.prim = b.prim;
      cap.dist = __float_as_uint(b.dist);
    }
    f3 N = f3{0.0f, 0.0f, 0.0f};
    wc.hits += (uint32_t)__popcll(__ballot(hit));
    bool zero = false;
    if (hit) {
      const float* nm = p.nrm + 9 * (size_t)b.prim;
      float w0 = 1.0f - b.u - b.v;
      N = add(add(scale(ld3(nm), w0), scale(ld3(nm + 3), b.u)), scale(ld3(nm + 6), b.v));
      zero = is_zero(N);
    }
    wc.zero_normal += (uint32_t)__popcll(__ballot(zero));
    hit = hit && !zero;
    const uint64_t hm = __ballot(hit);
    if (hm == 0) break;
    uint32_t base = 0;
    if (w.lane == 0) base = atomicAdd(p.hit_count + RT_HIT_STRIDE * x, (uint32_t)__popcll(hm));
    base = uni(base);
    bool deep = false;
    if (hit) {
      const uint32_t slot = base + (uint32_t)__popcll(hm & ((1ull << w.lane) - 1ull));
      const f3 P = hit_point(r, b.t);
      if (slot < p.hit_cap) {
        const size_t a = (size_t)x * p.hit_cap + slot;
        p.hit[2 * a] = make_float4(P.x, P.y, P.z, N.x);
        p.hit[2 * a + 1] = make_float4(N.y, N.z, coef, __uint_as_float(b.obj));
        p.hit_prev[a] = prev;
      }
      prev = x | (slot << 3);
      if (kCapture && depth == 0) cap.first = prev;
      const float ncoef = p.mat[RT_MAT_FLOATS_D * (size_t)b.obj + 10] * coef;
      if (depth + 1 >= RT_MAX_BOUNCES) {
        deep = !((double)ncoef < 0.01);
      } else {
        d = bounce_dir(d, N);
        o = P;
        coef = ncoef;
      }
    }
    wc.overflow += (uint32_t)__popcll(__ballot(deep));
    alive = hit && depth + 1 < RT_MAX_BOUNCES;
    ++depth;
  }
  return prev;
}

template <int ACCEL, bool COUNT, int POL>
__global__ __launch_bounds__(64, RT_TRACE_MIN_WAVES) void trace_kernel(KParams p) {
  const int lane = threadIdx.x & 63;
  WorkCount wc = {};
  __shared__ float4 s_stack[ACCEL == RT_ACCEL_FLAT_D ? 1 : kStackArea];
  __shared__ float4 s_stage[ACCEL == RT_ACCEL_FLAT_D ? kStageFlat : kStageOct];
  const size_t gl = (size_t)blockIdx.x * 64 + (size_t)lane;
  Stack stk;
  stk.idx = (uint32_t*)s_stack;
  stk.tt = (float*)s_stack + kLdsStack * 64;
  stk.spill = p.spill + gl;
  stk.stride = gridDim.x * 64u;
  stk.lane = lane;
  stk.sp = 0;
  WaveCtx w;
  w.stk2 = s_stack;
  w.stkm = (uint64_t*)(s_stack + 2 * kStack2);
  w.stage = s_stage;
  w.lane = lane;
  const uint32_t nt = (uint32_t)p.ntiles_local;
  const uint32_t home = (uint32_t)blockIdx.x & 7u;
  uint32_t probe = 0;
  bool first = true;
  unsigned long long wave_cost = 0;
  const uint32_t n_heavy = p.n_heavy ? uni(*p.n_heavy) : 0u;
  for (;;) {
    const uint32_t x = (home + probe) & 7u;
    const uint32_t nx = nt > x ? (nt - x + 7u) / 8u : 0u;
    uint32_t q = 0;
    if (first) {
      q = (uint32_t)blockIdx.x >> 3;
      first = false;
    } else {
      if (lane == 0) q = atomicAdd(p.tile_counter + 32u * x, 1u);
      q = uni(q) + (gridDim.x - x + 7u) / 8u;
    }
    if (q >= 4u * nx) {
      if (++probe == 8u) break;
      continue;
    }
    const uint32_t pos = 8u * (q >> 2) + x;
    const uint32_t u = 4u * (p.tile_order ? p.tile_order[pos] : pos) + (q & 3u);
    const bool prio = pos < n_heavy;
    if (prio) __builtin_amdgcn_s_setprio(3);
    const unsigned long long c0 = (COUNT || p.item_cost) ? __builtin_readcyclecounter() : 0ull;
    const uint32_t ph0[3] = {wc.cy_cam, wc.cy_cand, wc.cy_sec};
    wc.sec_lane_nodes = wc.sec_lane_tris = 0;
    const uint32_t t = u >> 2;
    int smp;
    f3 point, dir;
    const bool valid = camera_sample(p, t, u & 3u, lane, smp, point, dir);
    wc.pixels += (uint32_t)__popcll(__ballot(valid && smp == 0));
    Capture cap;
    p.last[(size_t)u * 64 + lane] =
        trace_path<ACCEL, COUNT, POL>(p, valid, point, dir, x, stk, w, wc, t, cap, 0, 1.0f, RT_NO_REC);
    if (POL == RT_POLICY_GBUFFER)
      p.capture[(size_t)u * 64 + lane] = make_uint4(cap.prim, cap.dist, cap.first, cap.queries);
    if (prio) __builtin_amdgcn_s_setprio(0);
    if (p.item_cost && lane == 0) {
      const unsigned long long cy = __builtin_readcyclecounter() - c0;
      p.item_cost[u] = cy < 0xffffffffull ? (uint32_t)cy : 0xffffffffu;
      wave_cost += cy;
    }
    if (COUNT && p.tile_cycles && lane == 0) {
      const size_t items = 4 * (size_t)p.ntiles_local;
      const uint32_t ph1[3] = {wc.cy_cam, wc.cy_cand, wc.cy_sec};
      p.tile_cycles[u] = __builtin_readcyclecounter() - c0;
#pragma unroll
      for (int k2 = 0; k2 < 3; k2++) p.tile_cycles[u + (size_t)(k2 + 1) * items] = ph1[k2] - ph0[k2];
      p.tile_cycles[u + 4 * items] = wc.sec_lane_nodes;
      p.tile_cycles[u + 5 * items] = wc.sec_lane_tris;
    }
  }
  if (p.cost_sum && lane == 0 && wave_cost) atomicAdd(p.cost_sum, wave_cost);
  flush_counts(p, wc, lane);
}

static constexpr int kLaneStackArea = kLdsStack * 64 * 8 / 16;

template <int ACCEL, bool COUNT, int POL, bool RELIGHT = false>
__device__ __forceinline__ col shade_record(const KParams& p, bool valid, size_t a, Stack& s,
                                            WaveCtx& w, WorkCount& wc, uint32_t& lit0) {
  col acc = init_color(0.0f, 0.0f, 0.0f);
  uint32_t pend = 0;
  for (uint32_t l0 = 0; l0 < p.nlight; l0 += 32) {
    const uint32_t l1 = p.nlight - l0 < 32u ? p.nlight : l0 + 32u;
    uint32_t lit = 0;
    if constexpr (RELIGHT)
      if (valid && l0 == 0) lit = p.hit_lit[a] & ~p.relight_dirty;
    {
      f3 P{0.0f, 0.0f, 0.0f};
      if (valid) {
        const float4 r0 = p.hit[2 * a];
        P = f3{r0.x, r0.y, r0.z};
      }
      for (uint32_t li = l0; li < l1; li++) {
        const float* L = p.light + RT_LIGHT_FLOATS_D * li;
        const uint32_t type = __float_as_uint(L[0]);
        if (type != 1 && type != 2) continue;
        if constexpr (RELIGHT)
          if (l0 == 0 && !((p.relight_dirty >> li) & 1u)) continue;
        const f3 lv = f3{L[4], L[5], L[6]};
        const uint64_t c0 = COUNT ? __builtin_readcyclecounter() : 0ull;
        bool df = false;
        const bool sh = shadow_q<ACCEL, COUNT, POL>(p, P, shadow_dir(type, lv, P), type, li, valid, s, w, wc,
                                                    &df, nullptr, l0 == 0);
        if (COUNT) {
          const uint32_t dc = (uint32_t)(__builtin_readcyclecounter() - c0);
          wc.cy_shadow += dc;
          if (type == 1) wc.cy_shadow_dir += dc;
        }
        if (df) pend |= 1u << li;
        if (!sh) lit |= 1u << (li - l0);
      }
    }
    if (l0 == 0) lit0 = lit;
    if (valid && pend && l0 == 0) {
      const uint32_t q = atomicAdd(p.oob_count, 1u);
      if (q < p.oob_cap) p.oob[q] = make_uint4((uint32_t)a, pend, lit & ~pend, 0u);
    }
    if (!valid) continue;
    const float4 r0 = p.hit[2 * a], r1 = p.hit[2 * a + 1];
    const f3 P{r0.x, r0.y, r0.z}, N{r0.w, r1.x, r1.y};
    const float* m = p.mat + RT_MAT_FLOATS_D * (size_t)__float_as_uint(r1.w);
    acc = lights_sum(p.light, acc, l0, l1, lit, m, P, N);
  }
  return acc;
}

template <int ACCEL, bool COUNT, int POL, bool RELIGHT = false>
__global__ __launch_bounds__(64, ACCEL == RT_ACCEL_FLAT_D ? RT_FLAT_SHADE_MIN_WAVES
                                : ((POL == RT_POLICY_STAGED || POL == RT_POLICY_DIR_STAGED) ? RT_STAGED_SHADE_MIN_WAVES
                                                                                              : RT_SHADE_MIN_WAVES)) void shade_kernel(KParams p) {
  const int lane = threadIdx.x & 63;
  WorkCount wc = {};
  constexpr bool kStaged = POL == RT_POLICY_STAGED || POL == RT_POLICY_DIR_STAGED;
  __shared__ float4 s_stack[ACCEL == RT_ACCEL_FLAT_D ? 1 : (kStaged ? kStackArea : kLaneStackArea)];
  __shared__ float4 s_stage[ACCEL == RT_ACCEL_FLAT_D ? kStageFlat : (kStaged ? kStageOct : 1)];
  const size_t gl = (size_t)blockIdx.x * 64 + (size_t)lane;
  Stack stk;
  stk.idx = (uint32_t*)s_stack;
  stk.tt = (float*)s_stack + kLdsStack * 64;
  stk.spill = p.spill + gl;
  stk.stride = gridDim.x * 64u;
  stk.lane = lane;
  stk.sp = 0;
  WaveCtx w;
  w.stk2 = s_stack;
  w.stkm = (uint64_t*)(s_stack + 2 * kStack2);
  w.stage = s_stage;
  w.lane = lane;
  const uint32_t home = (uint32_t)blockIdx.x & 7u;
  uint32_t probe = 0;
  bool first_chunk = true;
  for (;;) {
    const uint32_t x = (home + probe) & 7u;
    const uint32_t hc = p.hit_count[RT_HIT_STRIDE * x];
    const uint32_t n = hc < p.hit_cap ? hc : p.hit_cap;
    const uint32_t stride = p.shade_stride > 1u ? p.shade_stride : 1u;
    const uint32_t first = p.shade_first;
    const uint32_t ns = n > first ? (n - first + stride - 1u) / stride : 0u;
    uint32_t q = 0;
    if (first_chunk) {
      q = (uint32_t)blockIdx.x >> 3;
      first_chunk = false;
    } else {
      if (lane == 0) q = atomicAdd(p.shade_counter + RT_HIT_STRIDE * x, 1u);
      q = uni(q) + (gridDim.x - x + 7u) / 8u;
    }
    if (q >= (ns + 63u) / 64u) {
      if (++probe == 8u) break;
      continue;
    }
    const uint32_t k = q * 64u + (uint32_t)lane;
    const bool valid = k < ns;
    const size_t a = (size_t)x * p.hit_cap + (size_t)k * stride + first;
    uint32_t lit = 0;
    const col local = shade_record<ACCEL, COUNT, POL, RELIGHT>(p, valid, a, stk, w, wc, lit);
    if (valid) {
      const col tm = color_mul(local, p.hit[2 * a + 1].z);
      p.hit_term[a] = make_float4(tm.r, tm.g, tm.b, 0.0f);
      if (p.hit_lit) p.hit_lit[a] = lit;
    }
  }
  flush_counts(p, wc, lane, true);
}

static constexpr uint32_t kFixChunk = 16384;
static constexpr uint32_t kFixBatch = 64;
__device__ __forceinline__ uint32_t oob_queries(const KParams& p, uint32_t n) {
  if (n > kFixBatch) return kFixBatch + 1;
  uint32_t m = 0;
  for (uint32_t e = 0; e < n; e++) m += (uint32_t)__popc(p.oob[e].y & (p.nlight >= 32 ? 0xffffffffu : (1u << p.nlight) - 1u));
  return m;
}
__global__ __launch_bounds__(256) void oob_fix_kernel(KParams p, uint32_t nprim) {
  __shared__ uint32_t bits, skip, nqs;
  const uint32_t n = min(*p.oob_count, p.oob_cap);
  if (threadIdx.x == 0) nqs = oob_queries(p, n);
  __syncthreads();
  if (nqs <= kFixBatch) return;
  const uint32_t chunks = (nprim + kFixChunk - 1) / kFixChunk;
  for (uint64_t item = blockIdx.x; item < (uint64_t)n * chunks; item += gridDim.x) {
    const uint32_t e = (uint32_t)(item / chunks), c = (uint32_t)(item % chunks);
    const uint4 q = p.oob[e];
    if (threadIdx.x == 0) {
      bits = 0;
      skip = (__atomic_load_n(&p.oob[e].w, __ATOMIC_RELAXED) & q.y) == q.y;
    }
    __syncthreads();
    if (skip) {
      __syncthreads();
      continue;
    }
    const float4 r0 = p.hit[2 * (size_t)q.x];
    const f3 P{r0.x, r0.y, r0.z};
    uint32_t mine = 0, risk = 0;
    for (uint32_t li = 0; li < 32 && li < p.nlight; li++) {
      if (!((q.y >> li) & 1u)) continue;
      const float* L = p.light + RT_LIGHT_FLOATS_D * li;
      const uint32_t type = __float_as_uint(L[0]);
      const Ray r = make_ray(p, P, shadow_dir(type, f3{L[4], L[5], L[6]}, P), p.eps_rel);
      bool h = false;
      const uint32_t end = min(nprim, (c + 1) * kFixChunk);
      for (uint32_t k = c * kFixChunk + threadIdx.x; k < end && !h; k += blockDim.x) {
        const float4* t = p.tri_prim + 3 * (size_t)k;
        h = any_hit_rec(r, t[0], t[1], t[2], risk);
      }
      if (h) mine |= 1u << li;
    }
    if (mine) atomicOr(&bits, mine);
    if (risk) atomicAdd(p.stats + RT_ST_SHADOW_ZERO_RISK, 1ull);
    __syncthreads();
    if (threadIdx.x == 0 && bits) atomicOr(&p.oob[e].w, bits);
    __syncthreads();
  }
}

struct FixQuery {
  Ray r;
  uint32_t e, li;
};
__global__ __launch_bounds__(256) void oob_fix_batch_kernel(KParams p, uint32_t nprim) {
  __shared__ FixQuery qs[kFixBatch];
  __shared__ uint32_t nq;
  const uint32_t n = min(*p.oob_count, p.oob_cap);
  if (threadIdx.x == 0) {
    uint32_t m = 0;
    const bool batch = oob_queries(p, n) <= kFixBatch;
    for (uint32_t e = 0; e < n && batch; e++) {
      const uint4 q = p.oob[e];
      const float4 r0 = p.hit[2 * (size_t)q.x];
      const f3 P{r0.x, r0.y, r0.z};
      for (uint32_t li = 0; li < 32 && li < p.nlight; li++) {
        if (!((q.y >> li) & 1u) || m >= kFixBatch) continue;
        const float* L = p.light + RT_LIGHT_FLOATS_D * li;
        const uint32_t type = __float_as_uint(L[0]);
        qs[m].r = make_ray(p, P, shadow_dir(type, f3{L[4], L[5], L[6]}, P), p.eps_rel);
        qs[m].e = e;
        qs[m].li = li;
        m++;
      }
    }
    nq = m;
  }
  __syncthreads();
  const uint32_t m = nq;
  uint32_t risk = 0;
  for (uint32_t k = blockIdx.x * blockDim.x + threadIdx.x; k < nprim; k += gridDim.x * blockDim.x) {
    const float4* t = p.tri_prim + 3 * (size_t)k;
    const float4 a0 = t[0], a1 = t[1], a2 = t[2];
    for (uint32_t j = 0; j < m; j++) {
      const FixQuery& q = qs[j];
      if (any_hit_rec(q.r, a0, a1, a2, risk)) atomicOr(&p.oob[q.e].w, 1u << q.li);
    }
  }
  if (risk) atomicAdd(p.stats + RT_ST_SHADOW_ZERO_RISK, 1ull);
}

__global__ __launch_bounds__(64) void oob_reshade_kernel(KParams p) {
  const uint32_t n = min(*p.oob_count, p.oob_cap);
  for (uint32_t e = blockIdx.x * blockDim.x + threadIdx.x; e < n; e += gridDim.x * blockDim.x) {
    const uint4 q = p.oob[e];
    const size_t a = q.x;
    const uint32_t lit0 = q.z | (q.y & ~q.w);
    const float4 r0 = p.hit[2 * a], r1 = p.hit[2 * a + 1];
    const f3 P{r0.x, r0.y, r0.z}, N{r0.w, r1.x, r1.y};
    const float* m = p.mat + RT_MAT_FLOATS_D * (size_t)__float_as_uint(r1.w);
    const col acc =
        lights_sum(p.light, init_color(0.0f, 0.0f, 0.0f), 0, p.nlight < 32u ? p.nlight : 32u, lit0, m, P, N);
    const col tm = color_mul(acc, r1.z);
    p.hit_term[a] = make_float4(tm.r, tm.g, tm.b, 0.0f);
    if (p.hit_lit) p.hit_lit[a] = lit0;
  }
}

}

#include "rt_probe.h"

namespace rt {

__global__ __launch_bounds__(256) void fold_kernel(KParams p) {
  const uint32_t idx = blockIdx.x * blockDim.x + threadIdx.x;
  if (idx == 0 && p.frame_check) {
    uint32_t f = 0;
    for (int x = 0; x < RT_HIT_REGIONS; x++)
      if (p.hit_count[RT_HIT_STRIDE * x] > p.hit_cap) f |= RT_FRAME_HITBUF;
    unsigned long long s[RT_NSTATS] = {};
    for (int set = 0; set < RT_STAT_SETS; set++)
      for (int k = 0; k < RT_NSTATS; k++) s[k] += p.stats[set * RT_STAT_STRIDE + k];
    auto raised = [&s](uint32_t flag) {
      bool any = false;
      for (uint32_t k = 0; k < RT_NSTATS; k++) any = any || (rt_stat_frame_flag(k) == flag && s[k]);
      return any;
    };
    if (raised(RT_FRAME_DEPTH)) f |= RT_FRAME_DEPTH;
    if (raised(RT_FRAME_ZERO)) f |= RT_FRAME_ZERO;
    if (raised(RT_FRAME_UNPROVEN) || (p.oob_count && *p.oob_count > p.oob_cap)) f |= RT_FRAME_UNPROVEN;
    if (p.list_flag && *p.list_flag) f |= RT_FRAME_LISTS;
    atomicOr(p.frame_check, (unsigned long long)f);
    atomicAdd(p.frame_check + 1, 1ull);
    atomicAdd(p.frame_check + 2, s[RT_ST_CLOSEST]);
    atomicAdd(p.frame_check + 3, s[RT_ST_SHADOW]);
  }
  if (idx >= (uint32_t)p.ntiles_local * 64u) return;
  const uint32_t t = idx >> 6, lane = idx & 63u;
  int pr, pc;
  const int row = (int)(lane >> 3), col_ = (int)(lane & 7u);
  tile_pixel(p, t, row, col_, pr, pc);
  const int ii = p.W - pc, jj = p.H - pr;
  const bool valid = pr < p.H && pc < p.W && ii >= 1 && ii <= 2 * (p.W / 2) && jj >= 1 &&
                     jj <= 2 * (p.H / 2);
  const uint4 l4 = *(const uint4*)(p.last + rt_pixel_slots(t, row, col_));
  const uint32_t last[4] = {l4.x, l4.y, l4.z, l4.w};
  col acc = init_color(0.0f, 0.0f, 0.0f);
#pragma unroll
  for (int smp = 0; smp < 4; smp++) {
    col sc = init_color(0.0f, 0.0f, 0.0f);
    uint32_t r = last[smp];
    while (r != RT_NO_REC && (r >> 3) < p.hit_cap) {
      const size_t a = rec_addr(p, r);
      const float4 tm = p.hit_term[a];
      sc = color_add(sc, col{tm.x, tm.y, tm.z});
      r = p.hit_prev[a];
    }
    acc = color_add(acc, color_mul(sc, 0.25f));
  }
  if (!valid) acc = col{0.0f, 0.0f, 0.0f};
  float* o = p.out + (size_t)idx * 3;
  o[0] = acc.r;
  o[1] = acc.g;
  o[2] = acc.b;
}

}

#include "rt_compat.h"

namespace rt {

__global__ __launch_bounds__(256) void assemble_kernel(const float* __restrict__ tiles,
                                                       float* __restrict__ rgb, int W, int H,
                                                       int tiles_x, int ntiles, int nranks,
                                                       int tiles_per_rank) {
  size_t idx = (size_t)blockIdx.x * blockDim.x + threadIdx.x;
  size_t npx = (size_t)W * (size_t)H;
  if (idx >= npx) return;
  int row = (int)(idx / (size_t)W), col = (int)(idx % (size_t)W);
  uint32_t rank;
  const int tb = rt_block_side(nranks);
  const uint32_t local = rt_tile_local(col >> 3, row >> 3, (uint32_t)nranks,
                                       (uint32_t)rt_blocks_x(tiles_x, tb), (uint32_t)tb, &rank);
  int lane = ((row & 7) << 3) | (col & 7);
  const float* src = tiles + (((size_t)rank * tiles_per_rank + local) * 64 + lane) * 3;
  rgb[3 * idx + 0] = src[0];
  rgb[3 * idx + 1] = src[1];
  rgb[3 * idx + 2] = src[2];
  (void)ntiles;
}

__global__ __launch_bounds__(256) void assemble_words_kernel(const uint32_t* __restrict__ tiles,
                                                             uint32_t* __restrict__ out, int W, int H,
                                                             int tiles_x, int nranks, int tiles_per_rank,
                                                             int words) {
  const size_t idx = (size_t)blockIdx.x * blockDim.x + threadIdx.x;
  if (idx >= (size_t)W * (size_t)H * (size_t)words) return;
  const size_t px = idx / (size_t)words;
  const int k = (int)(idx % (size_t)words);
  const int row = (int)(px / (size_t)W), col = (int)(px % (size_t)W);
  uint32_t rank;
  const int tb = rt_block_side(nranks);
  const uint32_t local = rt_tile_local(col >> 3, row >> 3, (uint32_t)nranks,
                                       (uint32_t)rt_blocks_x(tiles_x, tb), (uint32_t)tb, &rank);
  const int lane = ((row & 7) << 3) | (col & 7);
  out[idx] = tiles[(((size_t)rank * tiles_per_rank + local) * 64 + lane) * (size_t)words + k];
}

__global__ __launch_bounds__(256) void gbuffer_kernel(KParams p, uint32_t* __restrict__ out) {
  const size_t g = (size_t)blockIdx.x * blockDim.x + threadIdx.x;
  if (g >= (size_t)p.ntiles_local * 256u) return;
  const uint32_t slot = (uint32_t)(g >> 2), smp = (uint32_t)g & 3u;
  const uint32_t t = slot >> 6, lane = slot & 63u;
  int pr, pc;
  const int row = (int)(lane >> 3), col_ = (int)(lane & 7u);
  tile_pixel(p, t, row, col_, pr, pc);
  const int ii = p.W - pc, jj = p.H - pr;
  const bool valid = pr < p.H && pc < p.W && ii >= 1 && ii <= 2 * (p.W / 2) && jj >= 1 &&
                     jj <= 2 * (p.H / 2);
  uint32_t prim = 0xffffffffu, obj = 0xffffffffu, queries = 0, dist = 0x7f800000u;
  float4 h0 = make_float4(0.0f, 0.0f, 0.0f, 0.0f), h1 = h0;
  if (valid) {
    const uint4 c = p.capture[rt_item_slot(t, row, col_, (int)smp)];
    queries = c.w;
    if (c.x != 0xffffffffu) {
      prim = c.x;
      dist = c.y;
      obj = __float_as_uint(p.tri_prim[3 * (size_t)prim + 2].z);
      if (c.z != RT_NO_REC && (c.z >> 3) < p.hit_cap) {
        const size_t a = rec_addr(p, c.z);
        h0 = p.hit[2 * a];
        h1 = p.hit[2 * a + 1];
      }
    }
  }
  uint2* o = (uint2*)(out + g * RT_GB_WORDS_D);
  o[0] = make_uint2(prim, obj);
  o[1] = make_uint2(queries, dist);
  o[2] = make_uint2(__float_as_uint(h0.x), __float_as_uint(h0.y));
  o[3] = make_uint2(__float_as_uint(h0.z), __float_as_uint(h0.w));
  o[4] = make_uint2(__float_as_uint(h1.x), __float_as_uint(h1.y));
}

}

#include "rt_recolour.h"

template <bool TRACE>
static const void* kernel_of(int accel, int count_work, int policy);

template <bool TRACE>
static const void* kernel_of(int accel, int count_work, int policy) {
  using namespace rt;
  if (TRACE && policy == RT_POLICY_GBUFFER)
    return accel == RT_ACCEL_FLAT_D ? (const void*)trace_kernel<RT_ACCEL_FLAT_D, false, RT_POLICY_GBUFFER>
                                    : (const void*)trace_kernel<RT_ACCEL_OCTREE_D, false, RT_POLICY_GBUFFER>;
  if (accel == RT_ACCEL_FLAT_D) {
    if (TRACE)
      return count_work ? (const void*)trace_kernel<RT_ACCEL_FLAT_D, true, 0>
                        : (const void*)trace_kernel<RT_ACCEL_FLAT_D, false, 0>;
    return count_work ? (const void*)shade_kernel<RT_ACCEL_FLAT_D, true, 0>
                      : (const void*)shade_kernel<RT_ACCEL_FLAT_D, false, 0>;
  }
  if (TRACE) {
    if (policy == RT_POLICY_EXACT_REFL)
      return count_work ? (const void*)trace_kernel<RT_ACCEL_OCTREE_D, true, RT_POLICY_EXACT_REFL>
                        : (const void*)trace_kernel<RT_ACCEL_OCTREE_D, false, RT_POLICY_EXACT_REFL>;
    if (policy == RT_POLICY_LANE) return (const void*)trace_kernel<RT_ACCEL_OCTREE_D, false, RT_POLICY_LANE>;
    if (policy == RT_POLICY_STAGED)
      return (const void*)trace_kernel<RT_ACCEL_OCTREE_D, false, RT_POLICY_STAGED>;
    return count_work ? (const void*)trace_kernel<RT_ACCEL_OCTREE_D, true, RT_POLICY_DEFAULT>
                      : (const void*)trace_kernel<RT_ACCEL_OCTREE_D, false, RT_POLICY_DEFAULT>;
  }
  if (policy == RT_POLICY_STAGED) return (const void*)shade_kernel<RT_ACCEL_OCTREE_D, false, RT_POLICY_STAGED>;
  if (policy == RT_POLICY_LBUF)
    return count_work ? (const void*)shade_kernel<RT_ACCEL_OCTREE_D, true, RT_POLICY_LBUF>
                      : (const void*)shade_kernel<RT_ACCEL_OCTREE_D, false, RT_POLICY_LBUF>;
  if (policy == RT_POLICY_DIR_STAGED)
    return (const void*)shade_kernel<RT_ACCEL_OCTREE_D, false, RT_POLICY_DIR_STAGED>;
  return count_work ? (const void*)shade_kernel<RT_ACCEL_OCTREE_D, true, RT_POLICY_DEFAULT>
                    : (const void*)shade_kernel<RT_ACCEL_OCTREE_D, false, RT_POLICY_DEFAULT>;
}

extern "C" hipError_t rt_render_grid(int trace, int accel, int count_work, int policy, int cus,
                                     int* grid) {
  const void* k = trace ? kernel_of<true>(accel, count_work, policy)
                        : kernel_of<false>(accel, count_work, policy);
  int per_cu = 0;
  hipError_t e = hipOccupancyMaxActiveBlocksPerMultiprocessor(&per_cu, k, 64, 0);
  if (e != hipSuccess) return e;
  if (per_cu < 1) per_cu = 1;
  if (per_cu > 32) per_cu = 32;
  *grid = per_cu * cus;
  return hipSuccess;
}

static hipError_t launch_kernel(const void* k, int grid, const KParams* p, hipStream_t stream) {
  void* args[] = {(void*)p};
  return hipLaunchKernel(k, dim3(grid), dim3(64), args, 0, stream);
}

extern "C" hipError_t rt_launch_trace(const KParams* p, int accel, int count_work, int policy,
                                      int grid, hipStream_t stream) {
  return launch_kernel(kernel_of<true>(accel, count_work, policy), grid, p, stream);
}

extern "C" hipError_t rt_launch_shade(const KParams* p, int accel, int count_work, int policy,
                                      int grid, hipStream_t stream) {
  return launch_kernel(kernel_of<false>(accel, count_work, policy), grid, p, stream);
}

extern "C" hipError_t rt_launch_shade_fixup(const KParams* p, uint32_t nprim, hipStream_t stream) {
  if (!p->oob) return hipGetLastError();
  hipLaunchKernelGGL(rt::oob_fix_batch_kernel, dim3(2048), dim3(256), 0, stream, *p, nprim);
  hipLaunchKernelGGL(rt::oob_fix_kernel, dim3(4096), dim3(256), 0, stream, *p, nprim);
  hipLaunchKernelGGL(rt::oob_reshade_kernel, dim3(64), dim3(64), 0, stream, *p);
  return hipGetLastError();
}

extern "C" hipError_t rt_launch_probe_shadow(const KParams* p, const float* org, uint32_t n, uint32_t li,
                                             uint32_t nprim, int brute, uint32_t* out, hipStream_t stream) {
  if (n == 0) return hipGetLastError();
  hipLaunchKernelGGL(rt::probe_shadow_kernel, dim3((n + 255) / 256), dim3(256), 0, stream, *p, org, n, li, nprim,
                     brute, out);
  return hipGetLastError();
}

extern "C" hipError_t rt_launch_probe_closest(const KParams* p, const float* org, const float* dir, uint32_t n,
                                              uint32_t nprim, int brute, uint32_t* out, int grid, hipStream_t stream) {
  if (n == 0) return hipSuccess;
  const uint32_t g = (n + 63) / 64;
  if (!brute && g > (uint32_t)grid) return hipErrorInvalidValue;
  hipLaunchKernelGGL(rt::probe_closest_kernel, dim3(g), dim3(64), 0, stream, *p, org, dir, n, nprim, brute, out);
  return hipGetLastError();
}

extern "C" hipError_t rt_launch_fold(const KParams* p, hipStream_t stream) {
  const uint32_t n = (uint32_t)p->ntiles_local * 64u;
  if (n == 0) return hipGetLastError();
  hipLaunchKernelGGL(rt::fold_kernel, dim3((n + 255) / 256), dim3(256), 0, stream, *p);
  return hipGetLastError();
}

extern "C" hipError_t rt_launch_assemble(const float* tiles, float* rgb, int W, int H, int tiles_x,
                                         int ntiles, int nranks, int tiles_per_rank,
                                         hipStream_t stream) {
  size_t npx = (size_t)W * (size_t)H;
  dim3 g((unsigned)((npx + 255) / 256)), b(256);
  hipLaunchKernelGGL(rt::assemble_kernel, g, b, 0, stream, tiles, rgb, W, H, tiles_x, ntiles,
                     nranks, tiles_per_rank);
  return hipGetLastError();
}

extern "C" hipError_t rt_launch_gbuffer(const KParams* p, uint32_t* out, hipStream_t stream) {
  const size_t n = (size_t)p->ntiles_local * 256u;
  if (n == 0) return hipGetLastError();
  hipLaunchKernelGGL(rt::gbuffer_kernel, dim3((unsigned)((n + 255) / 256)), dim3(256), 0, stream, *p, out);
  return hipGetLastError();
}

extern "C" hipError_t rt_launch_assemble_words(const uint32_t* tiles, uint32_t* out, int W, int H, int tiles_x,
                                               int nranks, int tiles_per_rank, int words,
                                               hipStream_t stream) {
  const size_t n = (size_t)W * (size_t)H * (size_t)words;
  if (n == 0) return hipGetLastError();
  if ((n + 255) / 256 > 0x7fffffffull) return hipErrorInvalidValue;
  hipLaunchKernelGGL(rt::assemble_words_kernel, dim3((unsigned)((n + 255) / 256)), dim3(256), 0, stream, tiles,
                     out, W, H, tiles_x, nranks, tiles_per_rank, words);
  return hipGetLastError();
}

extern "C" hipError_t rt_launch_compat(const KParams* p, int accel, int grid, hipStream_t stream) {
  dim3 g(grid), b(64);
  if (accel == RT_ACCEL_FLAT_D)
    hipLaunchKernelGGL((rt::compat_kernel<RT_ACCEL_FLAT_D, 0>), g, b, 0, stream, *p);
  else
    hipLaunchKernelGGL((rt::compat_kernel<RT_ACCEL_OCTREE_D, RT_POLICY_DEFAULT>), g, b, 0, stream, *p);
  return hipGetLastError();
}

extern "C" hipError_t rt_launch_downscale(const uint32_t* hi, uint32_t* lo, int W, int H,
                                          hipStream_t stream) {
  const int n = W * H;
  hipLaunchKernelGGL(rt::downscale_kernel, dim3((n + 255) / 256), dim3(256), 0, stream, hi, lo, W, H);
  return hipGetLastError();
}

extern "C" hipError_t rt_launch_relight_zero(const KParams* p, hipStream_t stream) {
  hipLaunchKernelGGL((rt::relight_zero_kernel<0>), dim3(1), dim3(256), 0, stream, *p);
  return hipGetLastError();
}

extern "C" hipError_t rt_launch_recolour(const KParams* p, int cus, hipStream_t stream) {
  const unsigned long long blocks = ((unsigned long long)p->hit_cap * RT_HIT_REGIONS + 255) / 256;
  const unsigned long long most = 8ull * (cus > 0 ? cus : 1);
  hipLaunchKernelGGL((rt::recolour_kernel<0>), dim3((unsigned)(blocks < most ? (blocks ? blocks : 1) : most)), dim3(256), 0,
                     stream, *p);
  return hipGetLastError();
}

extern "C" hipError_t rt_launch_reshade(const KParams* p, int accel, int policy, int grid, hipStream_t stream) {
  using namespace rt;
  const void* k = accel == RT_ACCEL_FLAT_D ? (const void*)shade_kernel<RT_ACCEL_FLAT_D, false, 0, true>
                  : policy == RT_POLICY_LBUF
                      ? (const void*)shade_kernel<RT_ACCEL_OCTREE_D, false, RT_POLICY_LBUF, true>
                      : (const void*)shade_kernel<RT_ACCEL_OCTREE_D, false, RT_POLICY_DEFAULT, true>;
  return launch_kernel(k, grid, p, stream);
}
```

### raytracing-gpu_amd/csrc/rt_shading.h

```cpp
#pragma once

#include "rt_query.h"

namespace rt {

#ifndef RT_SPEC_POW_INLINE
#define RT_SPEC_POW_INLINE __noinline__
#endif
__device__ RT_SPEC_POW_INLINE float spec_pow(double x, double e) { return (float)pow(fmax(x, 0.0), e); }

__device__ __forceinline__ col specular(col tmp, f3 inc_o, f3 inc_d, f3 P, f3 N, const float* m) {
  col k = init_color(m[6], m[7], m[8]);
  f3 V = sub(inc_o, P);
  f3 R = sub(inc_d, scale(N, 2.0f * dot(N, inc_d)));
  R = normalize(R);
  V = normalize(V);
  float ls = spec_pow((double)dot(R, V), (double)m[9]);
  k = color_mul(k, ls);
  return color_add(tmp, k);
}

__device__ __forceinline__ f3 shadow_dir(uint32_t type, f3 lv, f3 P) {
  return type == 1 ? scale(lv, -1.0f) : sub(lv, P);
}

__device__ __forceinline__ col light_lit(uint32_t type, col lc, f3 lv, const float* m, f3 P,
                                         f3 N) {
  if (type == 1) {
    f3 Ldir = scale(lv, -1.0f);
    col tmp = color_mul2(lc, init_color(m[3], m[4], m[5]));
    tmp = color_mul(tmp, dot(Ldir, N));
    f3 inc_o = add(P, scale(lv, -10.0f));
    return specular(tmp, inc_o, lv, P, N, m);
  }
  f3 to_l = sub(lv, P);
  f3 Lp = scale(lv, -1.0f);
  f3 Nf = N;
  if (dot(Lp, Nf) < 0.0f) Nf = scale(Nf, -1.0f);
  float dist = length(sub(lv, P));
  col tmp = color_mul2(lc, init_color(m[3], m[4], m[5]));
  tmp = color_mul(tmp, dot(Lp, Nf) * 1.0f / dist);
  f3 inc_o = add(P, scale(to_l, -10.0f));
  return specular(tmp, inc_o, to_l, P, N, m);
}

__device__ __forceinline__ col lights_sum(const float* light, col acc, uint32_t l0, uint32_t l1, uint32_t lit,
                                          const float* m, f3 P, f3 N) {
  for (uint32_t li = l0; li < l1; li++) {
    const float* L = light + RT_LIGHT_FLOATS_D * li;
    const uint32_t type = __float_as_uint(L[0]);
    const col lc = init_color(L[1], L[2], L[3]);
    if (type == 0)
      acc = color_add(acc, color_mul2(lc, init_color(m[0], m[1], m[2])));
    else if ((type == 1 || type == 2) && ((lit >> (li - l0)) & 1u))
      acc = color_add(acc, light_lit(type, lc, f3{L[4], L[5], L[6]}, m, P, N));
  }
  return acc;
}

template <int ACCEL, bool COUNT, int POL>
__device__ col apply_light(const KParams& p, bool hit, const float* m, f3 P, f3 N, Stack& s,
                           WaveCtx& w, WorkCount& wc) {
  col acc = init_color(0.0f, 0.0f, 0.0f);
  for (uint32_t li = 0; li < p.nlight; li++) {
    const float* L = p.light + RT_LIGHT_FLOATS_D * li;
    uint32_t type = __float_as_uint(L[0]);
    col lc = init_color(L[1], L[2], L[3]);
    f3 lv = f3{L[4], L[5], L[6]};
    if (type == 0) {
      if (hit) acc = color_add(acc, color_mul2(lc, init_color(m[0], m[1], m[2])));
    } else if (type == 1 || type == 2) {
      const uint64_t c0 = COUNT ? __builtin_readcyclecounter() : 0ull;
      bool sh = shadow_q<ACCEL, COUNT, POL>(p, P, shadow_dir(type, lv, P), type, li, hit, s, w, wc);
      if (COUNT) {
        const uint32_t dc = (uint32_t)(__builtin_readcyclecounter() - c0);
        wc.cy_shadow += dc;
        if (type == 1) wc.cy_shadow_dir += dc;
      }
      if (hit && !sh) acc = color_add(acc, light_lit(type, lc, lv, m, P, N));
    }
  }
  return acc;
}

}
```

Measured before the change: 9200 Mrays/s.

## Precompute per-light and per-material shading tables and hoist directional ray constants

Adds a small kernel that precomputes per-light rows (colour normalised to unit range, directional light length, unit direction and back-offset) and per-material rows with colours already divided by 255, and routes shading and shadow-ray construction through these tables. Directional shadow rays now reuse the precomputed length and unit direction instead of computing a sqrt and divides for every ray, and the unit direction is passed into the any-hit tests. Light-buffer descriptors are loaded through the scalar constant address space. The aim is less per-ray ALU work in shading and shadow setup, at the cost of extra device tables that must be rebuilt when lights or materials are edited, and possible small float differences from reordered colour multiplies.

```diff
diff --git a/raytracing-gpu_amd/csrc/rt_ctx.h b/raytracing-gpu_amd/csrc/rt_ctx.h
--- a/raytracing-gpu_amd/csrc/rt_ctx.h
+++ b/raytracing-gpu_amd/csrc/rt_ctx.h
@@ -75,6 +75,8 @@
   DevBuf<float> d_nrm;
   DevBuf<float> d_mat;
   DevBuf<float> d_light;
+  DevBuf<float> d_mshade;
+  DevBuf<float> d_lshade;
   DevBuf<float4> d_node;
   DevBuf<uint32_t> d_counter;
   unsigned long long* d_stats = nullptr;
@@ -216,6 +218,8 @@
   p.nrm = c->d_nrm;
   p.mat = c->d_mat;
   p.light = c->d_light;
+  p.mshade = c->d_mshade;
+  p.lshade = c->d_lshade;
   p.node = c->d_node;
   p.nrec = c->nrec;
   p.nlight = c->nlight;
diff --git a/raytracing-gpu_amd/csrc/rt_hip.cpp b/raytracing-gpu_amd/csrc/rt_hip.cpp
--- a/raytracing-gpu_amd/csrc/rt_hip.cpp
+++ b/raytracing-gpu_amd/csrc/rt_hip.cpp
@@ -27,6 +27,16 @@
 static int upload(DevBuf<T>& dst, const void* src, size_t bytes) {
   HIP_TRY(dst.alloc(bytes / sizeof(T)));
   if (src && bytes) HIP_TRY(hipMemcpy(dst, src, bytes, hipMemcpyHostToDevice));
+  return RT_OK;
+}
+
+static int shade_tables(rt_hip_ctx* c, bool lights, bool materials) {
+  const uint32_t nl = lights ? c->nlight : 0u;
+  const uint32_t no = materials ? (uint32_t)(c->mat_host.size() / RT_MAT_FLOATS) : 0u;
+  if (lights) HIP_TRY(c->d_lshade.alloc((size_t)nl * RT_LSHADE_FLOATS_D));
+  if (materials) HIP_TRY(c->d_mshade.alloc((size_t)no * RT_MAT_FLOATS));
+  HIP_TRY(rt_launch_shade_tables(c->d_light, nl, c->d_lshade, c->d_mat, no, c->d_mshade, c->stream));
+  HIP_TRY(hipStreamSynchronize(c->stream));
   return RT_OK;
 }
 
@@ -288,6 +298,7 @@
   c->info.build_seconds = std::chrono::duration<double>(dev_build ? t2 - t0 : t1 - t0).count();
   if (fs.mat) c->mat_host.assign(fs.mat, fs.mat + fs.nobj * RT_MAT_FLOATS);
   rt_flat_free(&fs);
+  if (!rc) rc = shade_tables(c, true, true);
   if (rc) {
     rt_hip_destroy(c);
     return rc;
@@ -876,6 +887,9 @@
   if (edited) c->sh_ulps = -1.0f;
   c->last_p.light = c->d_light;
   c->last_p.nlight = c->nlight;
+  rc = shade_tables(c, true, false);
+  c->last_p.lshade = c->d_lshade;
+  if (rc) return rc;
   if (!(c->light_buffers && c->accel == RT_ACCEL_OCTREE && c->d_node)) return RT_OK;
   const bool current = c->d_lbuf && c->lb_ulps == c->eps_ulps && c->lb_proven == c->exact_shadows &&
                        c->lb_dev.size() == old_n && c->lb_host.size() == old_n && c->lb_failed.size() == old_n;
@@ -941,7 +955,9 @@
   if (rc) return rc;
   HIP_TRY(hipMemcpy(c->d_mat, rows.data(), rows.size() * sizeof(float), hipMemcpyHostToDevice));
   c->mat_host = rows;
-  return RT_OK;
+  const int tables = shade_tables(c, false, true);
+  c->last_p.mshade = c->d_mshade;
+  return tables;
 }
 
 extern "C" int rt_hip_set_keep_visibility(rt_hip_ctx* c, int enable) {
@@ -972,6 +988,8 @@
     p.light = sp.light;
     p.nlight = sp.nlight;
     p.mat = sp.mat;
+    p.mshade = sp.mshade;
+    p.lshade = sp.lshade;
     p.eps_rel = sp.eps_rel;
     p.eps_rel_cam = sp.eps_rel_cam;
   }
@@ -997,7 +1015,8 @@
   if (w.path == RT_RELIGHT_RECOLOUR) p.oob = nullptr;
   if (!p.tri_prim && (p.lbuf || p.n_sh_global)) return rt_set_error(RT_EHIP, "relight: prim-order records missing");
   if (!p.hit || !p.hit_prev || !p.hit_term || !p.hit_lit || !p.hit_count || !p.shade_counter || !p.stats ||
-      !p.last || !p.out || (p.nlight && !p.light) || (p.nrec && (!p.tri || !p.nrm)) || !p.mat ||
+      !p.last || !p.out || (p.nlight && (!p.light || !p.lshade)) || (p.nrec && (!p.tri || !p.nrm)) || !p.mat ||
+      !p.mshade ||
       p.hit_cap != c->hit_cap() || !c->d_hit_lit.holds((size_t)p.hit_cap * RT_HIT_REGIONS))
     return rt_set_error(RT_EHIP, "relight: device buffers missing");
   HIP_TRY(rt_launch_relight_zero(&p, s));
diff --git a/raytracing-gpu_amd/csrc/rt_isect.h b/raytracing-gpu_amd/csrc/rt_isect.h
--- a/raytracing-gpu_amd/csrc/rt_isect.h
+++ b/raytracing-gpu_amd/csrc/rt_isect.h
@@ -39,17 +39,22 @@
   f3 oh, ol;
 };
 
-__device__ __forceinline__ Ray make_ray(const KParams& p, f3 o, f3 d, float eps_rel) {
+__device__ __forceinline__ Ray make_ray_len(const KParams& p, f3 o, f3 d, float dlen, float eps_rel) {
   Ray r;
   r.o = o;
   r.d = d;
-  r.dlen = length(d);
+  r.dlen = dlen;
   r.eps = rt_cull_eps(eps_rel, o.x - p.scene_c.x, o.y - p.scene_c.y, o.z - p.scene_c.z,
                       p.scene_cmag, p.scene_r);
   r.oh = f3{o.x + r.eps, o.y + r.eps, o.z + r.eps};
   r.ol = f3{o.x - r.eps, o.y - r.eps, o.z - r.eps};
   return r;
 }
+__device__ __forceinline__ Ray make_ray(const KParams& p, f3 o, f3 d, float eps_rel) {
+  return make_ray_len(p, o, d, length(d), eps_rel);
+}
+
+__device__ __forceinline__ f3 unit_dir(const Ray& r) { return f3{r.d.x / r.dlen, r.d.y / r.dlen, r.d.z / r.dlen}; }
 
 __device__ __forceinline__ f3 hit_point(const Ray& r, float t) {
   f3 nd{r.d.x / r.dlen, r.d.y / r.dlen, r.d.z / r.dlen};
@@ -58,6 +63,9 @@
 
 __device__ __forceinline__ float hit_dist(const Ray& r, float t) {
   return length(sub(hit_point(r, t), r.o));
+}
+__device__ __forceinline__ float hit_dist(const Ray& r, f3 nd, float t) {
+  return length(sub(add(r.o, scale(nd, t * r.dlen)), r.o));
 }
 
 __device__ __forceinline__ bool mt_candidate(f3 o, f3 d, f3 v0, f3 e1, f3 e2, float t_cut) {
@@ -163,24 +171,32 @@
   for (uint32_t k = 0; k < n; k++, k3 += 3) consider_w(r, act, am, stage[k3], stage[k3 + 1], stage[k3 + 2], b);
 }
 
-__device__ __forceinline__ bool any_hit_exact(const Ray& r, const float4& q0, const float4& q1,
+__device__ __forceinline__ bool any_hit_exact(const Ray& r, f3 nd, const float4& q0, const float4& q1,
                                               const float4& q2, uint32_t& risk);
 
+__device__ __forceinline__ bool any_hit_rec(const Ray& r, f3 nd, const float4& q0, const float4& q1,
+                                            const float4& q2, uint32_t& risk) {
+  f3 v0{q0.x, q0.y, q0.z}, e1{q0.w, q1.x, q1.y}, e2{q1.z, q1.w, q2.x};
+  if (!mt_candidate(r.o, r.d, v0, e1, e2, __builtin_inff())) return false;
+  return any_hit_exact(r, nd, q0, q1, q2, risk);
+}
 __device__ __forceinline__ bool any_hit_rec(const Ray& r, const float4& q0, const float4& q1,
                                             const float4& q2, uint32_t& risk) {
-  f3 v0{q0.x, q0.y, q0.z}, e1{q0.w, q1.x, q1.y}, e2{q1.z, q1.w, q2.x};
-  if (!mt_candidate(r.o, r.d, v0, e1, e2, __builtin_inff())) return false;
-  return any_hit_exact(r, q0, q1, q2, risk);
-}
-
+  return any_hit_rec(r, unit_dir(r), q0, q1, q2, risk);
+}
+
+__device__ __forceinline__ bool any_hit_exact(const Ray& r, f3 nd, const float4& q0, const float4& q1,
+                                              const float4& q2, uint32_t& risk) {
+  f3 v0{q0.x, q0.y, q0.z}, e1{q0.w, q1.x, q1.y}, e2{q1.z, q1.w, q2.x};
+  float t, u, v;
+  if (!mt_test(r.o, r.d, v0, e1, e2, t, u, v)) return false;
+  if (!((double)hit_dist(r, nd, t) > 0.01)) return false;
+  risk |= __float_as_uint(q2.w) & RT_REC_ZERO_RISK;
+  return true;
+}
 __device__ __forceinline__ bool any_hit_exact(const Ray& r, const float4& q0, const float4& q1,
                                               const float4& q2, uint32_t& risk) {
-  f3 v0{q0.x, q0.y, q0.z}, e1{q0.w, q1.x, q1.y}, e2{q1.z, q1.w, q2.x};
-  float t, u, v;
-  if (!mt_test(r.o, r.d, v0, e1, e2, t, u, v)) return false;
-  if (!((double)hit_dist(r, t) > 0.01)) return false;
-  risk |= __float_as_uint(q2.w) & RT_REC_ZERO_RISK;
-  return true;
-}
-
-}
+  return any_hit_exact(r, unit_dir(r), q0, q1, q2, risk);
+}
+
+}
diff --git a/raytracing-gpu_amd/csrc/rt_kernels.h b/raytracing-gpu_amd/csrc/rt_kernels.h
--- a/raytracing-gpu_amd/csrc/rt_kernels.h
+++ b/raytracing-gpu_amd/csrc/rt_kernels.h
@@ -11,6 +11,7 @@
 #define RT_ACCEL_OCTREE_D 1
 #define RT_MAT_FLOATS_D 12
 #define RT_LIGHT_FLOATS_D 8
+#define RT_LSHADE_FLOATS_D 16
 #define RT_MAX_BOUNCES 16384
 #define RT_SPILL_STACK 112
 #define RT_HIT_REGIONS 8
@@ -108,6 +109,8 @@
   const uint32_t* list_flag;
   uint4* capture;
   uint32_t relight_dirty;
+  const float* mshade;
+  const float* lshade;
 };
 
 extern "C" hipError_t rt_launch_trace(const KParams* p, int accel, int count_work, int policy,
@@ -119,6 +122,8 @@
 extern "C" hipError_t rt_launch_relight_zero(const KParams* p, hipStream_t stream);
 extern "C" hipError_t rt_launch_recolour(const KParams* p, int cus, hipStream_t stream);
 extern "C" hipError_t rt_launch_reshade(const KParams* p, int accel, int policy, int grid, hipStream_t stream);
+extern "C" hipError_t rt_launch_shade_tables(const float* light, uint32_t nlight, float* lshade, const float* mat,
+                                             uint32_t nobj, float* mshade, hipStream_t stream);
 extern "C" hipError_t rt_launch_probe_shadow(const KParams* p, const float* org, uint32_t n, uint32_t li,
                                              uint32_t nprim, int brute, uint32_t* out, hipStream_t stream);
 extern "C" hipError_t rt_launch_probe_closest(const KParams* p, const float* org, const float* dir, uint32_t n,
diff --git a/raytracing-gpu_amd/csrc/rt_query.h b/raytracing-gpu_amd/csrc/rt_query.h
--- a/raytracing-gpu_amd/csrc/rt_query.h
+++ b/raytracing-gpu_amd/csrc/rt_query.h
@@ -1,6 +1,7 @@
 #pragma once
 
 #include "rt_lightbuf_cell.h"
+#include "rt_shade_rows.h"
 #include "rt_walk_lane.h"
 #include "rt_walk_wave.h"
 
@@ -78,7 +79,8 @@
 }
 
 template <bool COUNT>
-__device__ bool lbuf_scan(const KParams& p, const RtLightBuf& L, const Ray& r, const LbRange& g, LaneCount& lc) {
+__device__ bool lbuf_scan(const KParams& p, const RtLightBuf& L, const Ray& r, f3 nd, const LbRange& g,
+                          LaneCount& lc) {
   for (int h = 0; h < 2; h++) {
     const float q = h == 0 ? g.lim : __builtin_inff();
     uint32_t k = g.rs[h];
@@ -103,7 +105,7 @@
         lc.tris += lanes_distinct(k);
         lc.ltris++;
       }
-      if (any_hit_rec(r, a0, a1, a2, lc.risk)) return true;
+      if (any_hit_rec(r, nd, a0, a1, a2, lc.risk)) return true;
     }
   }
   for (uint32_t k = 0; k < L.nglobal; k++) {
@@ -112,14 +114,25 @@
       lc.tris += lanes_distinct(L.global[k]);
       lc.ltris++;
     }
-    if (any_hit_rec(r, t[0], t[1], t[2], lc.risk)) return true;
+    if (any_hit_rec(r, nd, t[0], t[1], t[2], lc.risk)) return true;
   }
   return false;
 }
 
 template <bool COUNT>
 __device__ bool lbuf_any(const KParams& p, const RtLightBuf& L, const Ray& r, LaneCount& lc) {
-  return lbuf_scan<COUNT>(p, L, r, lbuf_range(L, r), lc);
+  return lbuf_scan<COUNT>(p, L, r, unit_dir(r), lbuf_range(L, r), lc);
+}
+
+__device__ __forceinline__ Ray lbuf_ray(const KParams& p, f3 o, f3 d, uint32_t type, uint32_t li, f3& nd) {
+  if (type == 1) {
+    const LightShade S = LightRowsUniform{p.lshade}[li];
+    nd = S.nd;
+    return make_ray_len(p, o, d, S.dlen, p.eps_rel);
+  }
+  const Ray r = make_ray(p, o, d, p.eps_rel);
+  nd = unit_dir(r);
+  return r;
 }
 
 template <int ACCEL, bool COUNT, int POL>
@@ -128,13 +141,16 @@
                                          const LbRange* pre = nullptr, bool can_defer = true) {
   uint64_t am = __ballot(act);
   wc.shadow += (uint32_t)__popcll(am);
-  Ray r = make_ray(p, o, d, p.eps_rel);
-  if (ACCEL == RT_ACCEL_FLAT_D)
+  if (ACCEL == RT_ACCEL_FLAT_D) {
+    const Ray r = make_ray(p, o, d, p.eps_rel);
     return use_tp(p, act) ? flat_any_tp<COUNT>(p, r, act, wc) : flat_any_w<COUNT>(p, r, act, w, wc);
+  }
   if (POL == RT_POLICY_LBUF) {
-    const RtLightBuf& L = p.lbuf[li];
-    LaneCount lc = {0, 0, 0, 0, 0, 0, 0, 0};
-    bool hit = act && (pre ? lbuf_scan<COUNT>(p, L, r, *pre, lc) : lbuf_any<COUNT>(p, L, r, lc));
+    const RtLightBuf L = lbuf_desc(p.lbuf, li);
+    f3 nd;
+    const Ray r = lbuf_ray(p, o, d, type, li, nd);
+    LaneCount lc = {0, 0, 0, 0, 0, 0, 0, 0};
+    bool hit = act && lbuf_scan<COUNT>(p, L, r, nd, pre ? *pre : lbuf_range(L, r), lc);
     absorb<COUNT>(wc, lc, true);
     if (L.proven) {
       const bool out = act && !(o.x >= L.olo[0] && o.x <= L.ohi[0] && o.y >= L.olo[1] && o.y <= L.ohi[1] &&
@@ -151,13 +167,15 @@
   bool staged = POL == RT_POLICY_STAGED ||
                 (POL == RT_POLICY_DIR_STAGED && type == 1 && __popcll(am) >= kPacketMin);
   bool hit, walked = true;
+  f3 nd;
+  const Ray r = lbuf_ray(p, o, d, type, li, nd);
   if (staged) {
     hit = staged_any<COUNT>(p, r, act, w, wc);
   } else if (p.lbuf && p.lbuf[li].kind != RT_LB_NONE) {
     walked = false;
     const RtLightBuf& L = p.lbuf[li];
     LaneCount lc = {0, 0, 0, 0, 0, 0, 0, 0};
-    hit = act && (pre ? lbuf_scan<COUNT>(p, L, r, *pre, lc) : lbuf_any<COUNT>(p, L, r, lc));
+    hit = act && lbuf_scan<COUNT>(p, L, r, nd, pre ? *pre : lbuf_range(L, r), lc);
     absorb<COUNT>(wc, lc, true);
     if (L.proven) {
       const bool out = act && !(o.x >= L.olo[0] && o.x <= L.ohi[0] && o.y >= L.olo[1] && o.y <= L.ohi[1] &&
diff --git a/raytracing-gpu_amd/csrc/rt_recolour.h b/raytracing-gpu_amd/csrc/rt_recolour.h
--- a/raytracing-gpu_amd/csrc/rt_recolour.h
+++ b/raytracing-gpu_amd/csrc/rt_recolour.h
@@ -25,22 +25,24 @@
 
 static constexpr uint32_t kRecolourLights = 64;
 
-__device__ __forceinline__ col recolour_sum(const float* light, uint32_t nlight, uint32_t mask, const float* m,
+template <class Rows>
+__device__ __forceinline__ col recolour_sum(const Rows& rows, uint32_t nlight, uint32_t mask, const float* ms,
                                             f3 P, f3 N) {
   col acc = init_color(0.0f, 0.0f, 0.0f);
   for (uint32_t l0 = 0; l0 < nlight; l0 += 32) {
     const uint32_t l1 = nlight - l0 < 32u ? nlight : l0 + 32u;
-    acc = lights_sum(light, acc, l0, l1, l0 == 0 ? mask : 0u, m, P, N);
+    acc = lights_sum(rows, acc, l0, l1, l0 == 0 ? mask : 0u, ms, P, N);
   }
   return acc;
 }
 
 template <int K = 0>
 __global__ __launch_bounds__(256) void recolour_kernel(KParams p) {
-  __shared__ float s_light[kRecolourLights * RT_LIGHT_FLOATS_D];
+  __shared__ float4 s_light[kRecolourLights * RT_LSHADE_FLOATS_D / 4];
   const bool staged = p.nlight <= kRecolourLights;
   if (staged)
-    for (uint32_t i = threadIdx.x; i < p.nlight * RT_LIGHT_FLOATS_D; i += blockDim.x) s_light[i] = p.light[i];
+    for (uint32_t i = threadIdx.x; i < p.nlight * (RT_LSHADE_FLOATS_D / 4); i += blockDim.x)
+      s_light[i] = ((const float4*)p.lshade)[i];
   __syncthreads();
   uint32_t end[RT_HIT_REGIONS];
   uint32_t total = 0;
@@ -64,9 +66,9 @@
     const float4 r0 = p.hit[2 * a], r1 = p.hit[2 * a + 1];
     const uint32_t mask = p.hit_lit[a];
     const f3 P{r0.x, r0.y, r0.z}, N{r0.w, r1.x, r1.y};
-    const float* m = p.mat + RT_MAT_FLOATS_D * (size_t)__float_as_uint(r1.w);
-    const col local = staged ? recolour_sum(s_light, p.nlight, mask, m, P, N)
-                             : recolour_sum(p.light, p.nlight, mask, m, P, N);
+    const float* ms = p.mshade + RT_MAT_FLOATS_D * (size_t)__float_as_uint(r1.w);
+    const col local = staged ? recolour_sum(LightRowsMem{s_light}, p.nlight, mask, ms, P, N)
+                             : recolour_sum(LightRowsUniform{p.lshade}, p.nlight, mask, ms, P, N);
     const col tm = color_mul(local, r1.z);
     p.hit_term[a] = make_float4(tm.r, tm.g, tm.b, 0.0f);
   }
diff --git a/raytracing-gpu_amd/csrc/rt_render.hip b/raytracing-gpu_amd/csrc/rt_render.hip
--- a/raytracing-gpu_amd/csrc/rt_render.hip
+++ b/raytracing-gpu_amd/csrc/rt_render.hip
@@ -247,12 +247,12 @@
         P = f3{r0.x, r0.y, r0.z};
       }
       for (uint32_t li = l0; li < l1; li++) {
-        const float* L = p.light + RT_LIGHT_FLOATS_D * li;
-        const uint32_t type = __float_as_uint(L[0]);
+        const LightShade L = LightRowsUniform{p.lshade}[li];
+        const uint32_t type = L.type;
         if (type != 1 && type != 2) continue;
         if constexpr (RELIGHT)
           if (l0 == 0 && !((p.relight_dirty >> li) & 1u)) continue;
-        const f3 lv = f3{L[4], L[5], L[6]};
+        const f3 lv = L.v;
         const uint64_t c0 = COUNT ? __builtin_readcyclecounter() : 0ull;
         bool df = false;
         const bool sh = shadow_q<ACCEL, COUNT, POL>(p, P, shadow_dir(type, lv, P), type, li, valid, s, w, wc,
@@ -274,8 +274,8 @@
     if (!valid) continue;
     const float4 r0 = p.hit[2 * a], r1 = p.hit[2 * a + 1];
     const f3 P{r0.x, r0.y, r0.z}, N{r0.w, r1.x, r1.y};
-    const float* m = p.mat + RT_MAT_FLOATS_D * (size_t)__float_as_uint(r1.w);
-    acc = lights_sum(p.light, acc, l0, l1, lit, m, P, N);
+    const float* ms = p.mshade + RT_MAT_FLOATS_D * (size_t)__float_as_uint(r1.w);
+    acc = lights_sum(LightRowsUniform{p.lshade}, acc, l0, l1, lit, ms, P, N);
   }
   return acc;
 }
@@ -370,9 +370,8 @@
     uint32_t mine = 0, risk = 0;
     for (uint32_t li = 0; li < 32 && li < p.nlight; li++) {
       if (!((q.y >> li) & 1u)) continue;
-      const float* L = p.light + RT_LIGHT_FLOATS_D * li;
-      const uint32_t type = __float_as_uint(L[0]);
-      const Ray r = make_ray(p, P, shadow_dir(type, f3{L[4], L[5], L[6]}, P), p.eps_rel);
+      const LightShade L = LightRowsUniform{p.lshade}[li];
+      const Ray r = make_ray(p, P, shadow_dir(L.type, L.v, P), p.eps_rel);
       bool h = false;
       const uint32_t end = min(nprim, (c + 1) * kFixChunk);
       for (uint32_t k = c * kFixChunk + threadIdx.x; k < end && !h; k += blockDim.x) {
@@ -406,9 +405,8 @@
       const f3 P{r0.x, r0.y, r0.z};
       for (uint32_t li = 0; li < 32 && li < p.nlight; li++) {
         if (!((q.y >> li) & 1u) || m >= kFixBatch) continue;
-        const float* L = p.light + RT_LIGHT_FLOATS_D * li;
-        const uint32_t type = __float_as_uint(L[0]);
-        qs[m].r = make_ray(p, P, shadow_dir(type, f3{L[4], L[5], L[6]}, P), p.eps_rel);
+        const LightShade L = LightRowsUniform{p.lshade}[li];
+        qs[m].r = make_ray(p, P, shadow_dir(L.type, L.v, P), p.eps_rel);
         qs[m].e = e;
         qs[m].li = li;
         m++;
@@ -438,9 +436,9 @@
     const uint32_t lit0 = q.z | (q.y & ~q.w);
     const float4 r0 = p.hit[2 * a], r1 = p.hit[2 * a + 1];
     const f3 P{r0.x, r0.y, r0.z}, N{r0.w, r1.x, r1.y};
-    const float* m = p.mat + RT_MAT_FLOATS_D * (size_t)__float_as_uint(r1.w);
-    const col acc =
-        lights_sum(p.light, init_color(0.0f, 0.0f, 0.0f), 0, p.nlight < 32u ? p.nlight : 32u, lit0, m, P, N);
+    const float* ms = p.mshade + RT_MAT_FLOATS_D * (size_t)__float_as_uint(r1.w);
+    const col acc = lights_sum(LightRowsUniform{p.lshade}, init_color(0.0f, 0.0f, 0.0f), 0,
+                               p.nlight < 32u ? p.nlight : 32u, lit0, ms, P, N);
     const col tm = color_mul(acc, r1.z);
     p.hit_term[a] = make_float4(tm.r, tm.g, tm.b, 0.0f);
     if (p.hit_lit) p.hit_lit[a] = lit0;
@@ -587,6 +585,7 @@
 }
 
 #include "rt_recolour.h"
+#include "rt_shade_tables.h"
 
 template <bool TRACE>
 static const void* kernel_of(int accel, int count_work, int policy);
@@ -749,3 +748,12 @@
                       : (const void*)shade_kernel<RT_ACCEL_OCTREE_D, false, RT_POLICY_DEFAULT, true>;
   return launch_kernel(k, grid, p, stream);
 }
+
+extern "C" hipError_t rt_launch_shade_tables(const float* light, uint32_t nlight, float* lshade, const float* mat,
+                                             uint32_t nobj, float* mshade, hipStream_t stream) {
+  const uint32_t n = nlight > nobj ? nlight : nobj;
+  if (!n) return hipSuccess;
+  hipLaunchKernelGGL((rt::shade_tables_kernel<0>), dim3((n + 255) / 256), dim3(256), 0, stream, light, nlight, lshade,
+                     mat, nobj, mshade);
+  return hipGetLastError();
+}
diff --git a/raytracing-gpu_amd/csrc/rt_shade_rows.h b/raytracing-gpu_amd/csrc/rt_shade_rows.h
--- /dev/null
+++ b/raytracing-gpu_amd/csrc/rt_shade_rows.h
@@ -0,0 +1,66 @@
+#pragma once
+
+#include "rt_kernels.h"
+#include "rt_walk_wave.h"
+
+namespace rt {
+
+struct LightShade {
+  uint32_t type;
+  float cr, cg, cb;
+  f3 v;
+  float dlen;
+  f3 nd, back;
+};
+
+__device__ __forceinline__ LightShade light_shade_of(const float4& a, const float4& b, const float4& c,
+                                                     const float4& d) {
+  LightShade s;
+  s.type = __float_as_uint(a.x);
+  s.cr = a.y, s.cg = a.z, s.cb = a.w;
+  s.v = f3{b.x, b.y, b.z};
+  s.dlen = b.w;
+  s.nd = f3{c.x, c.y, c.z};
+  s.back = f3{c.w, d.x, d.y};
+  return s;
+}
+__device__ __forceinline__ void light_shade_store(float* row, const LightShade& s) {
+  float4* r = (float4*)row;
+  r[0] = make_float4(__uint_as_float(s.type), s.cr, s.cg, s.cb);
+  r[1] = make_float4(s.v.x, s.v.y, s.v.z, s.dlen);
+  r[2] = make_float4(s.nd.x, s.nd.y, s.nd.z, s.back.x);
+  r[3] = make_float4(s.back.y, s.back.z, 0.0f, 0.0f);
+}
+
+struct LightRowsUniform {
+  const float* tab;
+  __device__ __forceinline__ LightShade operator[](uint32_t li) const {
+    const float4* r = (const float4*)tab + (RT_LSHADE_FLOATS_D / 4) * (size_t)li;
+    return light_shade_of(ldu(r, 0), ldu(r, 1), ldu(r, 2), ldu(r, 3));
+  }
+};
+struct LightRowsMem {
+  const float4* tab;
+  __device__ __forceinline__ LightShade operator[](uint32_t li) const {
+    const float4* r = tab + (RT_LSHADE_FLOATS_D / 4) * (size_t)li;
+    return light_shade_of(r[0], r[1], r[2], r[3]);
+  }
+};
+
+__device__ __forceinline__ RtLightBuf lbuf_desc(const RtLightBuf* lbuf, uint32_t li) {
+#if defined(__HIP_DEVICE_COMPILE__)
+  static_assert(sizeof(RtLightBuf) % sizeof(uint32_t) == 0, "copied word by word");
+  typedef const __attribute__((address_space(4))) uint32_t cword;
+  const cword* src = (const cword*)(lbuf + li);
+  uint32_t w[sizeof(RtLightBuf) / sizeof(uint32_t)];
+#pragma unroll
+  for (uint32_t k = 0; k < sizeof(RtLightBuf) / sizeof(uint32_t); k++) w[k] = src[k];
+  RtLightBuf L;
+  __builtin_memcpy(&L, w, sizeof L);
+  return L;
+#else
+  return lbuf[li];
+#endif
+}
+
+}
diff --git a/raytracing-gpu_amd/csrc/rt_shade_tables.h b/raytracing-gpu_amd/csrc/rt_shade_tables.h
--- /dev/null
+++ b/raytracing-gpu_amd/csrc/rt_shade_tables.h
@@ -0,0 +1,40 @@
+#pragma once
+
+#include "rt_shade_rows.h"
+
+namespace rt {
+
+template <int K = 0>
+__global__ __launch_bounds__(256) void shade_tables_kernel(const float* light, uint32_t nlight, float* lshade,
+                                                           const float* mat, uint32_t nobj, float* mshade) {
+  const uint32_t t = blockIdx.x * blockDim.x + threadIdx.x;
+  if (t < nlight) {
+    const float* L = light + RT_LIGHT_FLOATS_D * (size_t)t;
+    const col lc = init_color(L[1], L[2], L[3]);
+    LightShade s;
+    s.type = __float_as_uint(L[0]);
+    s.cr = lc.r / 255.0f, s.cg = lc.g / 255.0f, s.cb = lc.b / 255.0f;
+    s.v = f3{L[4], L[5], L[6]};
+    s.dlen = 0.0f;
+    s.nd = s.back = f3{0.0f, 0.0f, 0.0f};
+    if (s.type == 1) {
+      const f3 d = scale(s.v, -1.0f);
+      s.dlen = length(d);
+      s.nd = f3{d.x / s.dlen, d.y / s.dlen, d.z / s.dlen};
+      s.back = scale(s.v, -10.0f);
+    }
+    light_shade_store(lshade + RT_LSHADE_FLOATS_D * (size_t)t, s);
+  }
+  if (t < nobj) {
+    const float* m = mat + RT_MAT_FLOATS_D * (size_t)t;
+    float* ms = mshade + RT_MAT_FLOATS_D * (size_t)t;
+#pragma unroll
+    for (int g = 0; g < 3; g++) {
+      const col k = init_color(m[3 * g], m[3 * g + 1], m[3 * g + 2]);
+      ms[3 * g] = k.r / 255.0f, ms[3 * g + 1] = k.g / 255.0f, ms[3 * g + 2] = k.b / 255.0f;
+    }
+    ms[9] = m[9], ms[10] = m[10], ms[11] = m[11];
+  }
+}
+
+}
diff --git a/raytracing-gpu_amd/csrc/rt_shading.h b/raytracing-gpu_amd/csrc/rt_shading.h
--- a/raytracing-gpu_amd/csrc/rt_shading.h
+++ b/raytracing-gpu_amd/csrc/rt_shading.h
@@ -9,14 +9,13 @@
 #endif
 __device__ RT_SPEC_POW_INLINE float spec_pow(double x, double e) { return (float)pow(fmax(x, 0.0), e); }
 
-__device__ __forceinline__ col specular(col tmp, f3 inc_o, f3 inc_d, f3 P, f3 N, const float* m) {
-  col k = init_color(m[6], m[7], m[8]);
+__device__ __forceinline__ col specular(col tmp, f3 inc_o, f3 inc_d, f3 P, f3 N, const float* ms) {
   f3 V = sub(inc_o, P);
   f3 R = sub(inc_d, scale(N, 2.0f * dot(N, inc_d)));
   R = normalize(R);
   V = normalize(V);
-  float ls = spec_pow((double)dot(R, V), (double)m[9]);
-  k = color_mul(k, ls);
+  float ls = spec_pow((double)dot(R, V), (double)ms[9]);
+  col k = init_color(ms[6] * ls, ms[7] * ls, ms[8] * ls);
   return color_add(tmp, k);
 }
 
@@ -24,61 +23,34 @@
   return type == 1 ? scale(lv, -1.0f) : sub(lv, P);
 }
 
-__device__ __forceinline__ col light_lit(uint32_t type, col lc, f3 lv, const float* m, f3 P,
-                                         f3 N) {
-  if (type == 1) {
+__device__ __forceinline__ col light_lit(const LightShade& L, const float* ms, f3 P, f3 N) {
+  const f3 lv = L.v;
+  col tmp = init_color(L.cr * ms[3], L.cg * ms[4], L.cb * ms[5]);
+  if (L.type == 1) {
     f3 Ldir = scale(lv, -1.0f);
-    col tmp = color_mul2(lc, init_color(m[3], m[4], m[5]));
     tmp = color_mul(tmp, dot(Ldir, N));
-    f3 inc_o = add(P, scale(lv, -10.0f));
-    return specular(tmp, inc_o, lv, P, N, m);
+    f3 inc_o = add(P, L.back);
+    return specular(tmp, inc_o, lv, P, N, ms);
   }
   f3 to_l = sub(lv, P);
   f3 Lp = scale(lv, -1.0f);
   f3 Nf = N;
   if (dot(Lp, Nf) < 0.0f) Nf = scale(Nf, -1.0f);
   float dist = length(sub(lv, P));
-  col tmp = color_mul2(lc, init_color(m[3], m[4], m[5]));
   tmp = color_mul(tmp, dot(Lp, Nf) * 1.0f / dist);
   f3 inc_o = add(P, scale(to_l, -10.0f));
-  return specular(tmp, inc_o, to_l, P, N, m);
+  return specular(tmp, inc_o, to_l, P, N, ms);
 }
 
-__device__ __forceinline__ col lights_sum(const float* light, col acc, uint32_t l0, uint32_t l1, uint32_t lit,
-                                          const float* m, f3 P, f3 N) {
+template <class Rows>
+__device__ __forceinline__ col lights_sum(const Rows& rows, col acc, uint32_t l0, uint32_t l1, uint32_t lit,
+                                          const float* ms, f3 P, f3 N) {
   for (uint32_t li = l0; li < l1; li++) {
-    const float* L = light + RT_LIGHT_FLOATS_D * li;
-    const uint32_t type = __float_as_uint(L[0]);
-    const col lc = init_color(L[1], L[2], L[3]);
-    if (type == 0)
-      acc = color_add(acc, color_mul2(lc, init_color(m[0], m[1], m[2])));
-    else if ((type == 1 || type == 2) && ((lit >> (li - l0)) & 1u))
-      acc = color_add(acc, light_lit(type, lc, f3{L[4], L[5], L[6]}, m, P, N));
-  }
-  return acc;
-}
-
-template <int ACCEL, bool COUNT, int POL>
-__device__ col apply_light(const KParams& p, bool hit, const float* m, f3 P, f3 N, Stack& s,
-                           WaveCtx& w, WorkCount& wc) {
-  col acc = init_color(0.0f, 0.0f, 0.0f);
-  for (uint32_t li = 0; li < p.nlight; li++) {
-    const float* L = p.light + RT_LIGHT_FLOATS_D * li;
-    uint32_t type = __float_as_uint(L[0]);
-    col lc = init_color(L[1], L[2], L[3]);
-    f3 lv = f3{L[4], L[5], L[6]};
-    if (type == 0) {
-      if (hit) acc = color_add(acc, color_mul2(lc, init_color(m[0], m[1], m[2])));
-    } else if (type == 1 || type == 2) {
-      const uint64_t c0 = COUNT ? __builtin_readcyclecounter() : 0ull;
-      bool sh = shadow_q<ACCEL, COUNT, POL>(p, P, shadow_dir(type, lv, P), type, li, hit, s, w, wc);
-      if (COUNT) {
-        const uint32_t dc = (uint32_t)(__builtin_readcyclecounter() - c0);
-        wc.cy_shadow += dc;
-        if (type == 1) wc.cy_shadow_dir += dc;
-      }
-      if (hit && !sh) acc = color_add(acc, light_lit(type, lc, lv, m, P, N));
-    }
+    const LightShade L = rows[li];
+    if (L.type == 0)
+      acc = color_add(acc, init_color(L.cr * ms[0], L.cg * ms[1], L.cb * ms[2]));
+    else if ((L.type == 1 || L.type == 2) && ((lit >> (li - l0)) & 1u))
+      acc = color_add(acc, light_lit(L, ms, P, N));
   }
   return acc;
 }
```

Result: faster. 9574 Mrays/s (median of 6 runs) (+4.1%).
